# AMReX-Fluids/IAMR

Measured on AMD Instinct MI355X. Metric: cells-advanced/sec, higher is better.
Workload: dtype f64; 1 GPU; TaylorGreen 3D single level, one 256^3 box per GPU in a 1x1x1 arrangement (256x256x256 cells), periodic, nu=1e-4 cfl=0.7 Godunov_PLM be_cn_theta=0.5, full NavierStokes::advance per step

## Files before the change

iamr_amd/csrc/cabi.hip:

```cpp
#include "../../include/iamrx.h"
#include "operators.h"
#include "launch.h"
#include "amrns.h"
#include <string>
#include <cstring>
#include <vector>
#include <map>

using namespace iamrx;

struct iamrx_layout_s { LayoutP p; };
struct iamrx_mf_s { MultiFab mf; };

static thread_local std::string g_err;

#define IAMRX_TRY try {
#define IAMRX_CATCH                                                   \
    return 0; }                                                       \
    catch (const std::exception& e) { g_err = e.what(); return 1; }   \
    catch (...) { g_err = "unknown error"; return 2; }

static Geometry to_geom(const iamrx_geom* g)
{
    Geometry r;
// ... 565 lines not shown
        for (int d = 0; d < 3; ++d) { r[i].lo[d] = b ? b[6 * i + d] : 0; r[i].hi[d] = b ? b[6 * i + 3 + d] : 0; }
    return r;
}

int iamrx_mf_fill_physbc(iamrx_mf m, const iamrx_geom* g, int scomp, int ncomp, const int* bcrec, const double* edlo, const double* edhi)
{
    IAMRX_TRY
    auto bc = to_bcrec(bcrec, ncomp);
    fill_physbc_cc(to_geom(g), m->mf, scomp, ncomp, bc.data(), edlo, edhi);
    IAMRX_CATCH
}

int iamrx_godunov_extrap_vel_to_faces(const iamrx_geom* g, iamrx_mf vel, iamrx_mf force, iamrx_mf ux, iamrx_mf uy, iamrx_mf uz,
                                      double dt, const int* bcrec, int fit, int scheme)
{
    IAMRX_TRY
    auto bc = to_bcrec(bcrec, 3);
    MultiFab* um[3] = {&ux->mf, &uy->mf, &uz->mf};
    godunov_extrap_vel_to_faces(to_geom(g), vel->mf, force ? &force->mf : nullptr, um, dt, bc.data(), fit != 0, scheme);
    IAMRX_CATCH
}

int iamrx_godunov_compute_aofs(const iamrx_geom* g, iamrx_mf aofs, int acomp, iamrx_mf S, int ncomp, iamrx_mf force, iamrx_mf divu,
                               iamrx_mf ux, iamrx_mf uy, iamrx_mf uz, const int* iconserv, double dt, const int* bcrec,
                               int is_velocity, int fit, iamrx_mf ex, iamrx_mf ey, iamrx_mf ez, iamrx_mf fx, iamrx_mf fy, iamrx_mf fz, int scheme)
{
    IAMRX_TRY
    auto bc = to_bcrec(bcrec, ncomp);
    MultiFab* um[3] = {&ux->mf, &uy->mf, &uz->mf};
    MultiFab* ed[3] = {ex ? &ex->mf : nullptr, ey ? &ey->mf : nullptr, ez ? &ez->mf : nullptr};
    MultiFab* fl[3] = {fx ? &fx->mf : nullptr, fy ? &fy->mf : nullptr, fz ? &fz->mf : nullptr};
    godunov_compute_aofs(to_geom(g), aofs->mf, acomp, S->mf, ncomp, force ? &force->mf : nullptr, divu ? &divu->mf : nullptr, um,
                         iconserv, dt, bc.data(), is_velocity != 0, fit != 0, ex ? ed : nullptr, fx ? fl : nullptr, scheme);
    IAMRX_CATCH
}

int iamrx_nodal_residual(const iamrx_geom* g, iamrx_mf out, iamrx_mf phi, iamrx_mf sig, iamrx_mf rhs)
{
    IAMRX_TRY nodal_residual(to_geom(g), out->mf, phi->mf, sig->mf, rhs ? &rhs->mf : nullptr); IAMRX_CATCH
}
int iamrx_nodal_gs_color(const iamrx_geom* g, iamrx_mf phi, iamrx_mf rhs, iamrx_mf sig, int color)
{
    IAMRX_TRY nodal_gs_color(to_geom(g), phi->mf, rhs->mf, sig->mf, color); IAMRX_CATCH
}
int iamrx_nodal_gs_sweep(const iamrx_geom* g, iamrx_mf phi, iamrx_mf rhs, iamrx_mf sig, int fused)
{
    IAMRX_TRY
    Geometry gg = to_geom(g);
    if (fused == 3 || fused == 4) {
        static MultiFab& xb = *new MultiFab();
        if (!xb.defined() || xb.layout != phi->mf.layout || xb.ngrow != phi->mf.ngrow) xb.define(phi->mf.layout, node_type(), 1, phi->mf.ngrow);
        const bool wrap = fused == 4;
        if (wrap && !periodic_wrap_ok(gg, *phi->mf.layout, 4)) throw Error("iamrx_nodal_gs_sweep(4): not a single box spanning a periodic domain");
        const double cs = tune("BENCH_CSIG", 0.0);
        nodal_gs_fused_pass(gg, phi->mf, phi->mf, xb, rhs->mf, sig->mf, 0, wrap, nullptr, cs != 0.0 ? &cs : nullptr);
        nodal_gs_fused_pass(gg, phi->mf, xb, xb, rhs->mf, sig->mf, 1, wrap, nullptr, cs != 0.0 ? &cs : nullptr);
    } else if (fused == 2) {
        if (!nodal_smooth_small(gg, phi->mf, rhs->mf, sig->mf, 1)) throw Error("level does not qualify for the single-workgroup smoother");
        phi->mf.FillBoundary(gg);
    } else if (fused) {
        MultiFab xb(phi->mf.layout, node_type(), 1, phi->mf.ngrow);
        phi->mf.FillBoundary(gg);
        nodal_gs_fused_pass(gg, phi->mf, phi->mf, xb, rhs->mf, sig->mf, 0);
        xb.FillBoundary(gg);
        nodal_gs_fused_pass(gg, phi->mf, xb, xb, rhs->mf, sig->mf, 1);
        MultiFab::Copy(phi->mf, xb, 0, 0, 1, 0);
    } else {
        for (int c = 0; c < 8; ++c) { phi->mf.FillBoundary(gg); nodal_gs_color(gg, phi->mf, rhs->mf, sig->mf, c); }
    }
    IAMRX_CATCH
}
int iamrx_nodal_restrict(iamrx_mf c, iamrx_mf f) { IAMRX_TRY nodal_restrict(c->mf, f->mf); IAMRX_CATCH }
int iamrx_nodal_interp_add(iamrx_mf f, iamrx_mf c, iamrx_mf s) { IAMRX_TRY nodal_interp_add(f->mf, c->mf, s->mf); IAMRX_CATCH }
int iamrx_nodal_divu(const iamrx_geom* g, iamrx_mf rhs, iamrx_mf vel, int vcomp)
{
    IAMRX_TRY
    Geometry gg = to_geom(g);
    DomainBC bc;
    for (int d = 0; d < 3; ++d) bc.lo[d] = bc.hi[d] = gg.periodic[d] ? lo_periodic : lo_neumann;
    bc.maxorder = 2;
    nodal_divu(gg, rhs->mf, vel->mf, vcomp, &bc);
    IAMRX_CATCH
}
int iamrx_nodal_compgrad(const iamrx_geom* g, iamrx_mf gp, iamrx_mf phi)
{
    IAMRX_TRY nodal_mknewu(to_geom(g), nullptr, 0, phi->mf, nullptr, &gp->mf, false); IAMRX_CATCH
}

int iamrx_nodal_projection(const iamrx_geom* g, iamrx_mf vel, int vcomp, iamrx_mf phi, iamrx_mf sig, int sig_comp, const int lobc[3],
                           const int hibc[3], double rel_tol, double abs_tol, const iamrx_mg_opts* o, iamrx_mf gp, int increment_gp,
                           iamrx_mg_stats* st)
{
    IAMRX_TRY
    MGOpts op = to_opts(o);
    MGStats s = nodal_projection(to_geom(g), vel->mf, vcomp, phi->mf, sig->mf, sig_comp, to_bc(lobc, hibc, op.maxorder), rel_tol, abs_tol,
                                 op, gp ? &gp->mf : nullptr, increment_gp != 0);
    from_stats(s, st);
    IAMRX_CATCH
}

int iamrx_nodal_solve(const iamrx_geom* g, iamrx_mf phi, iamrx_mf rhs, iamrx_mf sig, int sig_comp, const int lobc[3], const int hibc[3],
                      double rel_tol, double abs_tol, const iamrx_mg_opts* o, iamrx_mg_stats* st)
{
    IAMRX_TRY
    MGOpts op = to_opts(o);
    NodalMG mg(to_geom(g), phi->mf.layout, to_bc(lobc, hibc, op.maxorder), op);
    mg.setSigma(sig->mf, sig_comp);
    MGStats s = mg.solve(phi->mf, rhs->mf, rel_tol, abs_tol);
    from_stats(s, st);
    IAMRX_CATCH
}

int iamrx_tensor_apply(const iamrx_geom* g, iamrx_mf out, iamrx_mf vel, double a, double b, iamrx_mf acoef, iamrx_mf ex, iamrx_mf ey,
                       iamrx_mf ez, const int* lobc, const int* hibc, int nbc, int maxorder)
{
    IAMRX_TRY
    IAMRX_ASSERT(nbc == 1 || nbc == 3);
    const MultiFab* eta[3] = {&ex->mf, &ey->mf, &ez->mf};
    DomainBC bcs[3];
    for (int n = 0; n < nbc; ++n) bcs[n] = to_bc(lobc + 3 * n, hibc + 3 * n, maxorder);
    tensor_apply(to_geom(g), out->mf, vel->mf, a, b, acoef ? &acoef->mf : nullptr, eta, bcs, nbc);
    IAMRX_CATCH
}

int iamrx_tensor_solve(const iamrx_geom* g, iamrx_mf soln, iamrx_mf rhs, double a, double b, iamrx_mf acoef, iamrx_mf ex, iamrx_mf ey,
                       iamrx_mf ez, const int* lobc, const int* hibc, int nbc, double tol_rel, double tol_abs, const iamrx_mg_opts* o,
                       iamrx_mg_stats* st)
{
    IAMRX_TRY
    IAMRX_ASSERT(nbc == 1 || nbc == 3);
    MGOpts op = to_opts(o);
    const MultiFab* eta[3] = {&ex->mf, &ey->mf, &ez->mf};
    DomainBC bcs[3];
    for (int n = 0; n < nbc; ++n) bcs[n] = to_bc(lobc + 3 * n, hibc + 3 * n, op.maxorder);
    MGStats s = tensor_solve(to_geom(g), soln->mf, rhs->mf, a, b, acoef ? &acoef->mf : nullptr, eta, bcs, nbc, tol_rel, tol_abs, op);
    from_stats(s, st);
    IAMRX_CATCH
}

int iamrx_tensor_extensive_flux(const iamrx_geom* g, iamrx_mf vel, iamrx_mf ex, iamrx_mf ey, iamrx_mf ez, iamrx_mf fx, iamrx_mf fy, iamrx_mf fz,
                                double fac, int add)
{
    IAMRX_TRY
    const MultiFab* eta[3] = {&ex->mf, &ey->mf, &ez->mf};
    MultiFab* fl[3] = {&fx->mf, &fy->mf, &fz->mf};
    tensor_extensive_flux(to_geom(g), vel->mf, eta, fl, fac, add != 0);
    IAMRX_CATCH
}

int iamrx_tensor_apply_cf(const iamrx_geom* g, iamrx_mf out, iamrx_mf vel, double a, double b, iamrx_mf acoef, iamrx_mf ex, iamrx_mf ey,
                          iamrx_mf ez, const int* lobc, const int* hibc, int nbc, int maxorder, iamrx_mf crse_vel, const iamrx_geom* cgeom, int ratio)
{
    IAMRX_TRY
    IAMRX_ASSERT(nbc == 1 || nbc == 3);
    const MultiFab* eta[3] = {&ex->mf, &ey->mf, &ez->mf};
    DomainBC bcs[3];
    for (int n = 0; n < nbc; ++n) bcs[n] = to_bc(lobc + 3 * n, hibc + 3 * n, maxorder);
    Geometry cg = to_geom(cgeom);
    TensorCF cf{crse_vel ? &crse_vel->mf : nullptr, &cg, ratio};
    tensor_apply(to_geom(g), out->mf, vel->mf, a, b, acoef ? &acoef->mf : nullptr, eta, bcs, nbc, &cf);
    IAMRX_CATCH
}

int iamrx_tensor_solve_cf(const iamrx_geom* g, iamrx_mf soln, iamrx_mf rhs, double a, double b, iamrx_mf acoef, iamrx_mf ex, iamrx_mf ey,
                          iamrx_mf ez, const int* lobc, const int* hibc, int nbc, iamrx_mf crse_vel, const iamrx_geom* cgeom, int ratio,
                          double tol_rel, double tol_abs, const iamrx_mg_opts* o, iamrx_mg_stats* st)
// ... 797 lines not shown
```

iamr_amd/csrc/k_basic.hip:

```cpp
#include "kernels.h"
#include "launch.h"

namespace iamrx {

__global__ void __launch_bounds__(256) k_fill(double* __restrict__ p, size_t n, double v)
{
    size_t i = (size_t)blockIdx.x * 256 + threadIdx.x;
    const size_t stride = (size_t)gridDim.x * 256;
    for (; i < n; i += stride) p[i] = v;
}

void launch_fill(double* p, size_t n, double v, hipStream_t s)
{
    if (n == 0) return;
    size_t nb = (n + 255) / 256;
    if (nb > 4096) nb = 4096;
    hipLaunchKernelGGL(k_fill, dim3((unsigned)nb), dim3(256), 0, s, p, n, v);
}

__global__ void __launch_bounds__(256) k_copy_plan(const CopyDesc* __restrict__ descs, const FabD* __restrict__ src,
                                                   const FabD* __restrict__ dst, int scomp, int dcomp, int nc, int add)
{
    const CopyDesc cd = descs[blockIdx.y];
    const int nx = cd.region.len(0), ny = cd.region.len(1);
    const long npts = cd.npts();
    const FabD s = src[cd.src_fab], d = dst[cd.dst_fab];
    for (long q = (long)blockIdx.x * 256 + threadIdx.x; q < npts; q += (long)gridDim.x * 256) {
        const int i = cd.region.lo[0] + (int)(q % nx);
        const long r = q / nx;
        const int j = cd.region.lo[1] + (int)(r % ny);
        const int k = cd.region.lo[2] + cd.kstep * (int)(r / ny);
        if (add) for (int n = 0; n < nc; ++n) d(i, j, k, dcomp + n) += s(i + cd.shift[0], j + cd.shift[1], k + cd.shift[2], scomp + n);
        else for (int n = 0; n < nc; ++n) d(i, j, k, dcomp + n) = s(i + cd.shift[0], j + cd.shift[1], k + cd.shift[2], scomp + n);
    }
}

void launch_copy_plan(const CopyDesc* d, int nd, long maxpts, const FabD* src, const FabD* dst, int scomp, int dcomp, int nc, hipStream_t s, bool add)
{
    if (nd == 0) return;
    long nb = (maxpts + 255) / 256;
    const long cap = nd >= 8 ? 256 : 4096;
    if (nb > cap) nb = cap;
    if (nb < 1) nb = 1;
    hipLaunchKernelGGL(k_copy_plan, dim3((unsigned)nb, (unsigned)nd), dim3(256), 0, s, d, src, dst, scomp, dcomp, nc, add ? 1 : 0);
}

__global__ void __launch_bounds__(256) k_pack(const CopyDesc* __restrict__ descs, const FabD* __restrict__ src,
                                              double* __restrict__ buf, long pts_total, int scomp, int nc)
{
    const CopyDesc cd = descs[blockIdx.y];
    const int nx = cd.region.len(0), ny = cd.region.len(1);
    const long npts = cd.npts();
    const FabD s = src[cd.src_fab];
    for (long q = (long)blockIdx.x * 256 + threadIdx.x; q < npts; q += (long)gridDim.x * 256) {
        const int i = cd.region.lo[0] + (int)(q % nx);
        const long r = q / nx;
        const int j = cd.region.lo[1] + (int)(r % ny);
        const int k = cd.region.lo[2] + cd.kstep * (int)(r / ny);
        for (int n = 0; n < nc; ++n) buf[cd.buf_off + q + pts_total * n] = s(i + cd.shift[0], j + cd.shift[1], k + cd.shift[2], scomp + n);
    }
}

__global__ void __launch_bounds__(256) k_unpack(const CopyDesc* __restrict__ descs, const FabD* __restrict__ dst,
                                                const double* __restrict__ buf, long pts_total, int dcomp, int nc, int add)
{
    const CopyDesc cd = descs[blockIdx.y];
    const int nx = cd.region.len(0), ny = cd.region.len(1);
    const long npts = cd.npts();
    const FabD d = dst[cd.dst_fab];
    for (long q = (long)blockIdx.x * 256 + threadIdx.x; q < npts; q += (long)gridDim.x * 256) {
        const int i = cd.region.lo[0] + (int)(q % nx);
        const long r = q / nx;
        const int j = cd.region.lo[1] + (int)(r % ny);
        const int k = cd.region.lo[2] + cd.kstep * (int)(r / ny);
        if (add) for (int n = 0; n < nc; ++n) d(i, j, k, dcomp + n) += buf[cd.buf_off + q + pts_total * n];
        else for (int n = 0; n < nc; ++n) d(i, j, k, dcomp + n) = buf[cd.buf_off + q + pts_total * n];
    }
}

void launch_pack(const CopyDesc* d, int nd, long maxpts, const FabD* src, double* buf, long pts_total, int scomp, int nc, hipStream_t s)
{
    if (nd == 0) return;
    long nb = (maxpts + 255) / 256; if (nb > 256) nb = 256; if (nb < 1) nb = 1;
    hipLaunchKernelGGL(k_pack, dim3((unsigned)nb, (unsigned)nd), dim3(256), 0, s, d, src, buf, pts_total, scomp, nc);
// ... 339 lines not shown
}

template <bool MASK>
__global__ void __launch_bounds__(256) k_sum_integrated(Tiling t, const BoxD* __restrict__ boxes, const FabD* __restrict__ st, const FabD* __restrict__ cov,
                                                        int rho_comp, int trac_comp, double* __restrict__ partials, int np)
{
    const int fab = tile_fab(t);
    const BoxD b = boxes[fab];
    int i, j, k0, k1;
    double s0 = 0.0, s1 = 0.0, s2 = 0.0;
    if (tile_ijk(t, b, i, j, k0, k1)) {
        const FabD s = st[fab];
        for (int k = k0; k <= k1; ++k) {
            if (MASK && cov[fab](i, j, k) != 0.0) continue;
            const double u = s(i, j, k, 0), v = s(i, j, k, 1), w = s(i, j, k, 2), r = s(i, j, k, rho_comp), q = s(i, j, k, trac_comp);
            s0 += r; s1 += q; s2 += 0.5 * r * (u * u + v * v + w * w);
        }
    }
    const size_t slot = (size_t)blockIdx.y * gridDim.x + blockIdx.x;
    s0 = block_reduce<0>(s0);
    if (threadIdx.x == 0) partials[slot] = s0;
    s1 = block_reduce<0>(s1);
    if (threadIdx.x == 0) partials[(size_t)np + slot] = s1;
    s2 = block_reduce<0>(s2);
    if (threadIdx.x == 0) partials[2 * (size_t)np + slot] = s2;
}

void reduce_sum_integrated(const MultiFab& S, int rho_comp, int trac_comp, const MultiFab* cov, double out[3])
{
    IAMRX_ASSERT(S.type.cell() && (!cov || (cov->type.cell() && cov->layout->id == S.layout->id)));
    out[0] = out[1] = out[2] = 0.0;
    if (S.nlocal() == 0) return;
    auto& ctx = Context::get();
    Tiling t = level_tiling(*S.layout, S.type, 0, 8, true);
    dim3 g = t.grid();
    const int np = (int)(g.x * g.y);
    ctx.ensure_scratch((size_t)3 * np + 16);
    if (cov) hipLaunchKernelGGL((k_sum_integrated<true>), g, Tiling::block(), 0, ctx.stream, t, S.layout->d_boxes, S.d_tab, cov->d_tab, rho_comp, trac_comp, ctx.d_scratch, np);
    else hipLaunchKernelGGL((k_sum_integrated<false>), g, Tiling::block(), 0, ctx.stream, t, S.layout->d_boxes, S.d_tab, (const FabD*)nullptr, rho_comp, trac_comp, ctx.d_scratch, np);
    finish_to_host(0, 3, np, false);
    for (int q = 0; q < 3; ++q) out[q] = ctx.h_scratch[q];
}

void mf_lincomb(MultiFab& dst, double a, const MultiFab& x, double b, const MultiFab& y, int comp, int nc, int ng)
{
    trace_blas_site("lincomb", dst.layout ? dst.layout->local_cells() * nc : 0);
    if (!dst.base) return;
    const FabD *dt = dst.d_tab, *xt = x.d_tab, *yt = y.d_tab;
    for_each_2ph(*dst.layout, dst.type, ng, nc, Context::get().stream,
        [=] __device__(int i, int j, int k, int f, int n) { return a * xt[f](i, j, k, comp + n) + b * yt[f](i, j, k, comp + n); },
        [=] __device__(int i, int j, int k, int f, int n, double v) { dt[f](i, j, k, comp + n) = v; });
}

void mf_saxpy(MultiFab& y, double a, const MultiFab& x, int xcomp, int ycomp, int nc, int ng)
{
    trace_blas_site("saxpy", y.layout ? y.layout->local_cells() * nc : 0);
    if (!y.base) return;
    const FabD *yt = y.d_tab, *xt = x.d_tab;
    for_each_2ph(*y.layout, y.type, ng, nc, Context::get().stream,
        [=] __device__(int i, int j, int k, int f, int n) { return yt[f](i, j, k, ycomp + n) + a * xt[f](i, j, k, xcomp + n); },
        [=] __device__(int i, int j, int k, int f, int n, double v) { yt[f](i, j, k, ycomp + n) = v; });
}

void mf_add_scalar(MultiFab& y, double a, int comp, int nc, int ng)
{
    if (!y.base) return;
    const FabD* yt = y.d_tab;
    for_each(*y.layout, y.type, ng, Context::get().stream, [=] __device__(int i, int j, int k, int f) {
        const FabD yy = yt[f];
        for (int n = 0; n < nc; ++n) yy(i, j, k, comp + n) += a;
    });
}

void mf_mult(MultiFab& y, double a, int comp, int nc, int ng)
{
    trace_blas_site("mult", y.layout ? y.layout->local_cells() * nc : 0);
    if (!y.base) return;
    const FabD* yt = y.d_tab;
    for_each_2ph(*y.layout, y.type, ng, nc, Context::get().stream,
        [=] __device__(int i, int j, int k, int f, int n) { return yt[f](i, j, k, comp + n) * a; },
        [=] __device__(int i, int j, int k, int f, int n, double v) { yt[f](i, j, k, comp + n) = v; });
}

void slab_duplicate(MultiFab& dst, const MultiFab& src)
{
    IAMRX_ASSERT(dst.ncomp == src.ncomp && dst.layout->boxes.size() == src.layout->boxes.size());
    if (dst.nlocal() == 0) return;
    const FabD *dt = dst.d_tab, *st = src.d_tab;
    const int nc = dst.ncomp;
    for_each(*dst.layout, dst.type, 0, Context::get().stream, [=] __device__(int i, int j, int k, int f) {
        const FabD s = st[f];
        for (int n = 0; n < nc; ++n) dt[f](i, j, k, n) = s(i, 0, k, n);
    });
}

}
```

iamr_amd/csrc/k_nodal.hip:

```cpp
#include "kernels.h"
#include <cstring>
#include <type_traits>
#include "launch.h"

namespace iamrx {

struct NodeW { double corner, ex, ey, ez, fx, fy, fz, c; };

static NodeW make_w(const Geometry& g)
{
    const double fx = 1.0 / (g.dx[0] * g.dx[0]) / 36.0, fy = 1.0 / (g.dx[1] * g.dx[1]) / 36.0, fz = 1.0 / (g.dx[2] * g.dx[2]) / 36.0;
    NodeW w;
    w.corner = fx + fy + fz;
    w.ex = -fx + 2.0 * fy + 2.0 * fz;
    w.ey = 2.0 * fx - fy + 2.0 * fz;
    w.ez = 2.0 * fx + 2.0 * fy - fz;
    w.fx = 4.0 * fx - 2.0 * fy - 2.0 * fz;
    w.fy = -2.0 * fx + 4.0 * fy - 2.0 * fz;
    w.fz = -2.0 * fx - 2.0 * fy + 4.0 * fz;
    w.c = -4.0 * (fx + fy + fz);
    return w;
}

__device__ __forceinline__ double node_Ax(const FabD& x, const FabD& s, const NodeW& w, int i, int j, int k, double& s0)
// ... 1300 lines not shown
    long M = 1;
    for (int d = 0; d < 3; ++d) {
        if (b.len(d) < 2 || b.len(d) > 8) return false;
        G.wrap[d] = (g.periodic[d] && b.lo[d] == g.domain.lo[d] && b.hi[d] == g.domain.hi[d]) ? 1 : 0;
        G.m[d] = b.len(d) + (G.wrap[d] ? 0 : 1);
        G.lo[d] = b.lo[d]; G.n[d] = b.len(d);
        G.half_lo[d] = g.half_lo[d]; G.half_hi[d] = g.half_hi[d]; G.dlo[d] = g.domain.lo[d]; G.dhi[d] = g.domain.hi[d];
        M *= G.m[d];
    }
    return M <= NBG_NT;
}

bool nodal_bottom_device_ok_general(const Geometry& g, const Layout& l)
{
    const bool enabled = tune("MG_DEVICE_BOTTOM", 1) != 0 && tune("MG_DEVICE_BOTTOM_GENERAL", 1) != 0;
    NBotGeom G;
    return enabled && nbg_geom(g, l, G);
}

void nodal_bottom_solve_general(const Geometry& g, MultiFab& cor, const MultiFab& res, const MultiFab& sig, const MultiFab* dmask, bool singular,
                                double eps_rel, int maxiter, int nsweeps, int nub, int nuf, int* d_iters)
{
    const Layout& l = *cor.layout;
    NBotGeom G;
    IAMRX_ASSERT(nbg_geom(g, l, G) && sig.ngrow >= 1);
    if (l.nlocal() == 0) return;
    double cnt = 1.0;
    for (int d = 0; d < 3; ++d) cnt *= (double)g.domain.len(d);
    hipLaunchKernelGGL(k_nodal_bottom_g, dim3(1), dim3(NBG_NT), 0, Context::get().stream, cor.d_tab, res.d_tab, sig.d_tab,
                       dmask ? dmask->d_tab : nullptr, make_w(g), G, singular ? 1 : 0, cnt, eps_rel, maxiter, nsweeps, nub, nuf, d_iters);
}

void nodal_jacobi(const Geometry& g, MultiFab& xnew, const MultiFab& x, const MultiFab& rhs, const MultiFab& sig, const MultiFab* dmask)
{
    if (x.nlocal() == 0) return;
    const NodeW w = make_w(g);
    const FabD *nt = xnew.d_tab, *xt = x.d_tab, *rt = rhs.d_tab, *st = sig.d_tab, *dt = dmask ? dmask->d_tab : nullptr;
    for_each(*x.layout, node_type(), 0, Context::get().stream, [=] __device__(int i, int j, int k, int f) {
        if (dt && dt[f](i, j, k) != 0.0) { nt[f](i, j, k) = xt[f](i, j, k); return; }
        double s0;
        const double Ax = node_Ax(xt[f], st[f], w, i, j, k, s0);
        nt[f](i, j, k) = xt[f](i, j, k) + (2. / 3.) * (rt[f](i, j, k) - Ax) / s0;
    });
}

void nodal_zero_masked(MultiFab& mf, const MultiFab& dmask)
{
    if (mf.nlocal() == 0) return;
    const FabD *mt = mf.d_tab, *dt = dmask.d_tab;
    for_each(*mf.layout, node_type(), 0, Context::get().stream, [=] __device__(int i, int j, int k, int f) {
        if (dt[f](i, j, k) != 0.0) mt[f](i, j, k) = 0.0;
    });
}

void nodal_build_dmask(const Geometry& g, MultiFab& dm, const MultiFab& cov, const DomainBC& bc)
{
    if (dm.nlocal() == 0) return;
    const FabD *dt = dm.d_tab, *ct = cov.d_tab;
    int lo[3], hi[3], tlo[3], thi[3];
    for (int d = 0; d < 3; ++d) {
        lo[d] = g.domain.lo[d]; hi[d] = g.domain.hi[d];
        tlo[d] = g.periodic[d] ? 0 : bc.lo[d]; thi[d] = g.periodic[d] ? 0 : bc.hi[d];
    }
    const int l0 = lo[0], l1 = lo[1], l2 = lo[2], h0 = hi[0], h1 = hi[1], h2 = hi[2];
    const int a0 = tlo[0], a1 = tlo[1], a2 = tlo[2], b0 = thi[0], b1 = thi[1], b2 = thi[2];
    for_each(*dm.layout, node_type(), 0, Context::get().stream, [=] __device__(int i, int j, int k, int f) {
        const FabD c = ct[f];
        bool in = true;
        for (int q = 0; q < 8; ++q) {
            int ci = i - 1 + (q & 1), cj = j - 1 + ((q >> 1) & 1), ck = k - 1 + ((q >> 2) & 1);
            bool out = false;
            if (ci < l0) { if (a0 == lo_neumann) ci = 2 * l0 - 1 - ci; else if (a0 != 0) out = true; }
            else if (ci > h0) { if (b0 == lo_neumann) ci = 2 * h0 + 1 - ci; else if (b0 != 0) out = true; }
            if (cj < l1) { if (a1 == lo_neumann) cj = 2 * l1 - 1 - cj; else if (a1 != 0) out = true; }
            else if (cj > h1) { if (b1 == lo_neumann) cj = 2 * h1 + 1 - cj; else if (b1 != 0) out = true; }
            if (ck < l2) { if (a2 == lo_neumann) ck = 2 * l2 - 1 - ck; else if (a2 != 0) out = true; }
            else if (ck > h2) { if (b2 == lo_neumann) ck = 2 * h2 + 1 - ck; else if (b2 != 0) out = true; }
            if (out || c(ci, cj, ck) == 0.0) in = false;
        }
        dt[f](i, j, k) = in ? 0.0 : 1.0;
    });
}

void nodal_restrict(MultiFab& crse, const MultiFab& fine)
{
    if (crse.nlocal() == 0) return;
    const FabD *ct = crse.d_tab, *ft = fine.d_tab;
    for_each(*crse.layout, node_type(), 0, Context::get().stream, [=] __device__(int i, int j, int k, int f) {
        const FabD fa = ft[f];
        const int ii = 2 * i, jj = 2 * j, kk = 2 * k;
        double s = 0.0;
        for (int dk = -1; dk <= 1; ++dk)
            for (int dj = -1; dj <= 1; ++dj)
                for (int di = -1; di <= 1; ++di) {
                    const double w = (di == 0 ? 2. : 1.) * (dj == 0 ? 2. : 1.) * (dk == 0 ? 2. : 1.);
                    s += w * fa(ii + di, jj + dj, kk + dk);
                }
        ct[f](i, j, k) = s * (1. / 64.);
    });
}

#ifndef IAMRX_INTERP_EXP
#define IAMRX_INTERP_EXP 0
#endif
__device__ __forceinline__ double w_side(const FabD& s, int i, int j, int k, int d, int side)
{
    int lo[3] = {i - 1, j - 1, k - 1}, hi[3] = {i, j, k};
    lo[d] = hi[d] = (d == 0 ? i : (d == 1 ? j : k)) - 1 + side;
    double r = 0.0;
    for (int c = lo[2]; c <= hi[2]; ++c) for (int b = lo[1]; b <= hi[1]; ++b) for (int a = lo[0]; a <= hi[0]; ++a) r += s(a, b, c);
    return r;
}
__device__ __forceinline__ double interp_line(const FabD& c, const FabD& s, int i, int j, int k, int ic, int jc, int kc, int d)
{
    const double w1 = w_side(s, i, j, k, d, 0), w2 = w_side(s, i, j, k, d, 1);
    const double c2 = c(ic + (d == 0), jc + (d == 1), kc + (d == 2));
    return (c(ic, jc, kc) * w1 + c2 * w2) / (w1 + w2);
}
__device__ __forceinline__ double interp_face(const FabD& c, const FabD& s, int i, int j, int k, int ic, int jc, int kc, int d1, int d2)
{
    const double w1 = w_side(s, i, j, k, d1, 0), w2 = w_side(s, i, j, k, d1, 1), w3 = w_side(s, i, j, k, d2, 0), w4 = w_side(s, i, j, k, d2, 1);
    const int e1[3] = {d1 == 0, d1 == 1, d1 == 2}, e2[3] = {d2 == 0, d2 == 1, d2 == 2};
    double r = 0.0;
    r += w1 * interp_line(c, s, i - e1[0], j - e1[1], k - e1[2], ic, jc, kc, d2);
    r += w2 * interp_line(c, s, i + e1[0], j + e1[1], k + e1[2], ic + e1[0], jc + e1[1], kc + e1[2], d2);
    r += w3 * interp_line(c, s, i - e2[0], j - e2[1], k - e2[2], ic, jc, kc, d1);
    r += w4 * interp_line(c, s, i + e2[0], j + e2[1], k + e2[2], ic + e2[0], jc + e2[1], kc + e2[2], d1);
    return r / (w1 + w2 + w3 + w4);
}

template <class SA>
__device__ __forceinline__ void side_weights(const SA& s, int i, int j, int k, double w[6])
{
#if IAMRX_INTERP_EXP & 1
    for (int t = 0; t < 6; ++t) w[t] = 1.0 + 1e-3 * t;
    return;
#endif
    double g[2][2][2];
#pragma unroll
    for (int c = 0; c < 2; ++c)
#pragma unroll
        for (int b = 0; b < 2; ++b)
#pragma unroll
            for (int a = 0; a < 2; ++a) g[c][b][a] = s(i - 1 + a, j - 1 + b, k - 1 + c);
#pragma unroll
    for (int t = 0; t < 2; ++t) {
        w[t] = ((g[0][0][t] + g[0][1][t]) + g[1][0][t]) + g[1][1][t];
        w[2 + t] = ((g[0][t][0] + g[0][t][1]) + g[1][t][0]) + g[1][t][1];
        w[4 + t] = ((g[t][0][0] + g[t][0][1]) + g[t][1][0]) + g[t][1][1];
    }
}

template <int PX, int PY, int PZ, int CX, int CY, int CZ, class SA>
__device__ __forceinline__ void interp_class(double (*T)[2 * CY + 1][2 * CX + 1], const FabD& c, const SA& s, int fi0, int fj0, int fk0,
                                             int nhi0, int nhi1, int nhi2, int tid)
{
    constexpr int NX = PX ? CX : CX + 1, NY = PY ? CY : CY + 1, NZ = PZ ? CZ : CZ + 1, CLS = PX + PY + PZ;
    for (int idx = tid; idx < NX * NY * NZ; idx += 256) {
        const int lx = 2 * (idx % NX) + PX, q = idx / NX, ly = 2 * (q % NY) + PY, lz = 2 * (q / NY) + PZ;
        const int i = fi0 + lx, j = fj0 + ly, k = fk0 + lz;
        if (i > nhi0 || j > nhi1 || k > nhi2) continue;
        if (CLS == 0) { T[lz][ly][lx] = c(i >> 1, j >> 1, k >> 1); continue; }
        double w[6];
        side_weights(s, i, j, k, w);
        if (CLS == 1) {
            constexpr int d = PX ? 0 : (PY ? 1 : 2);
            const double w1 = w[2 * d], w2 = w[2 * d + 1];
            T[lz][ly][lx] = (IAMRX_INTERP_EXP & 4) ? (T[lz - PZ][ly - PY][lx - PX] * w1 + T[lz + PZ][ly + PY][lx + PX] * w2) * (w1 + w2) : (T[lz - PZ][ly - PY][lx - PX] * w1 + T[lz + PZ][ly + PY][lx + PX] * w2) / (w1 + w2);
        } else if (CLS == 2) {
            constexpr int d1 = PX ? 0 : 1, d2 = PZ ? 2 : 1;
// ... 16 lines not shown
__global__ void __launch_bounds__(256) k_nodal_interp_lds(const BoxD* __restrict__ fboxes, const FabD* __restrict__ ft, const FabD* __restrict__ ct,
    const FabD* __restrict__ st, int ntx, int nty)
{
    constexpr int FX = 2 * CX + 1, FY = 2 * CY + 1, FZ = 2 * CZ + 1, NF = FX * FY * FZ;
    __shared__ double T[FZ][FY][FX];
    const int fab = blockIdx.y;
    const BoxD vb = fboxes[fab];
    const int bid = blockIdx.x;
    const int tix = bid % ntx, r1 = bid / ntx, tiy = r1 % nty, tiz = r1 / nty;
    const int nhi0 = vb.hi[0] + 1, nhi1 = vb.hi[1] + 1, nhi2 = vb.hi[2] + 1;
    const int fi0 = vb.lo[0] + tix * 2 * CX, fj0 = vb.lo[1] + tiy * 2 * CY, fk0 = vb.lo[2] + tiz * 2 * CZ;
    if (fi0 >= nhi0 || fj0 >= nhi1 || fk0 >= nhi2) return;
    const FabD c = ct[fab], sg = st[fab], fa = ft[fab];
    const int tid = threadIdx.x;
    const FabD& s = sg;
#define IAMRX_ICLS(PX, PY, PZ) interp_class<PX, PY, PZ, CX, CY, CZ>(T, c, s, fi0, fj0, fk0, nhi0, nhi1, nhi2, tid)
    IAMRX_ICLS(0, 0, 0);
    __syncthreads();
    IAMRX_ICLS(1, 0, 0); IAMRX_ICLS(0, 1, 0); IAMRX_ICLS(0, 0, 1);
    __syncthreads();
    IAMRX_ICLS(1, 1, 0); IAMRX_ICLS(1, 0, 1); IAMRX_ICLS(0, 1, 1);
    __syncthreads();
    IAMRX_ICLS(1, 1, 1);
    __syncthreads();
#undef IAMRX_ICLS
    for (int idx = tid; idx < NF; idx += 256) {
        const int lx = idx % FX, q = idx / FX, ly = q % FY, lz = q / FY;
        const int i = fi0 + lx, j = fj0 + ly, k = fk0 + lz;
        if (i > nhi0 || j > nhi1 || k > nhi2) continue;
        if ((lx == 2 * CX && i != nhi0) || (ly == 2 * CY && j != nhi1) || (lz == 2 * CZ && k != nhi2)) continue;
        if (IAMRX_INTERP_EXP & 2) fa(i, j, k) = T[lz][ly][lx]; else fa(i, j, k) += T[lz][ly][lx];
    }
}

static bool nodal_interp_lds_enabled()
{
    const bool on = tune("NODAL_INTERP_LDS", 1) != 0;
    return on;
}

void nodal_interp_add(MultiFab& fine, const MultiFab& crse, const MultiFab& sig_fine)
{
    if (fine.nlocal() == 0) return;
    if (nodal_interp_lds_enabled()) {
        const Layout& l = *fine.layout;
        bool even = true;
        for (int d = 0; d < 3; ++d) even = even && l.all_lo_even[d];
        if (even) {
            constexpr int CX = 16, CY = 4, CZ = 4;
            const int ntx = (l.max_len[0] + 2 * CX - 1) / (2 * CX), nty = (l.max_len[1] + 2 * CY - 1) / (2 * CY), ntz = (l.max_len[2] + 2 * CZ - 1) / (2 * CZ);
            dim3 grid((unsigned)(ntx * nty * ntz), (unsigned)l.nlocal());
            hipLaunchKernelGGL((k_nodal_interp_lds<CX, CY, CZ>), grid, dim3(256), 0, Context::get().stream, l.d_boxes, fine.d_tab, crse.d_tab, sig_fine.d_tab, ntx, nty);
            return;
        }
    }
    const FabD *ft = fine.d_tab, *ct = crse.d_tab, *st = sig_fine.d_tab;
    const BoxD* fb = fine.layout->d_boxes;
    for_each(*crse.layout, node_type(), 0, Context::get().stream, [=] __device__(int ic, int jc, int kc, int f) {
        const FabD c = ct[f], s = st[f], fa = ft[f];
        const BoxD vb = fb[f];
        const int nhi0 = vb.hi[0] + 1, nhi1 = vb.hi[1] + 1, nhi2 = vb.hi[2] + 1;
        const int i0 = 2 * ic, j0 = 2 * jc, k0 = 2 * kc;
        const bool xi = i0 + 1 <= nhi0, xj = j0 + 1 <= nhi1, xk = k0 + 1 <= nhi2;
        fa(i0, j0, k0) += c(ic, jc, kc);
        if (xi) fa(i0 + 1, j0, k0) += interp_line(c, s, i0 + 1, j0, k0, ic, jc, kc, 0);
        if (xj) fa(i0, j0 + 1, k0) += interp_line(c, s, i0, j0 + 1, k0, ic, jc, kc, 1);
        if (xk) fa(i0, j0, k0 + 1) += interp_line(c, s, i0, j0, k0 + 1, ic, jc, kc, 2);
        if (xi && xj) fa(i0 + 1, j0 + 1, k0) += interp_face(c, s, i0 + 1, j0 + 1, k0, ic, jc, kc, 0, 1);
        if (xi && xk) fa(i0 + 1, j0, k0 + 1) += interp_face(c, s, i0 + 1, j0, k0 + 1, ic, jc, kc, 0, 2);
        if (xj && xk) fa(i0, j0 + 1, k0 + 1) += interp_face(c, s, i0, j0 + 1, k0 + 1, ic, jc, kc, 1, 2);
        if (xi && xj && xk) {
            const int i = i0 + 1, j = j0 + 1, k = k0 + 1;
            double w[6];
            for (int d = 0; d < 3; ++d) { w[2 * d] = w_side(s, i, j, k, d, 0); w[2 * d + 1] = w_side(s, i, j, k, d, 1); }
            const double v = (w[0] * interp_face(c, s, i - 1, j, k, ic, jc, kc, 1, 2) + w[1] * interp_face(c, s, i + 1, j, k, ic + 1, jc, kc, 1, 2)
               + w[2] * interp_face(c, s, i, j - 1, k, ic, jc, kc, 0, 2) + w[3] * interp_face(c, s, i, j + 1, k, ic, jc + 1, kc, 0, 2)
               + w[4] * interp_face(c, s, i, j, k - 1, ic, jc, kc, 0, 1) + w[5] * interp_face(c, s, i, j, k + 1, ic, jc, kc + 1, 0, 1))
              / (w[0] + w[1] + w[2] + w[3] + w[4] + w[5]);
            fa(i, j, k) += v;
        }
    });
}

void nodal_divu(const Geometry& g, MultiFab& rhs, const MultiFab& vel, int vcomp, const DomainBC* bc)
{
    if (rhs.nlocal() == 0) return;
    const FabD *rt = rhs.d_tab, *vt = vel.d_tab;
    const double fx = 0.25 / g.dx[0], fy = 0.25 / g.dx[1], fz = 0.25 / g.dx[2];
    int wl[3], wh[3], il[3], ih[3];
    for (int d = 0; d < 3; ++d) {
        wl[d] = (bc && !g.periodic[d] && bc->lo[d] == lo_neumann) ? 1 : 0;
        wh[d] = (bc && !g.periodic[d] && bc->hi[d] == lo_neumann) ? 1 : 0;
        il[d] = (bc && !g.periodic[d] && bc->lo[d] == lo_inflow) ? 1 : 0;
        ih[d] = (bc && !g.periodic[d] && bc->hi[d] == lo_inflow) ? 1 : 0;
    }
    const int wl0 = wl[0], wl1 = wl[1], wl2 = wl[2], wh0 = wh[0], wh1 = wh[1], wh2 = wh[2];
    const int il0 = il[0], il1 = il[1], il2 = il[2], ih0 = ih[0], ih1 = ih[1], ih2 = ih[2];
    const int dl0 = g.domain.lo[0], dl1 = g.domain.lo[1], dl2 = g.domain.lo[2], dh0 = g.domain.hi[0], dh1 = g.domain.hi[1], dh2 = g.domain.hi[2];
    for_each(*rhs.layout, node_type(), 0, Context::get().stream, [=] __device__(int i, int j, int k, int f) {
        const FabD v = vt[f];
        double sx = 0.0, sy = 0.0, sz = 0.0;
        for (int cz = 0; cz < 2; ++cz) for (int cy = 0; cy < 2; ++cy) for (int cx = 0; cx < 2; ++cx) {
            const int ci = i - 1 + cx, cj = j - 1 + cy, ck = k - 1 + cz;
            const bool outside = (wl0 && ci < dl0) || (wh0 && ci > dh0) || (wl1 && cj < dl1) || (wh1 && cj > dh1) || (wl2 && ck < dl2) || (wh2 && ck > dh2);
            const bool in0 = (il0 && ci < dl0) || (ih0 && ci > dh0), in1 = (il1 && cj < dl1) || (ih1 && cj > dh1), in2 = (il2 && ck < dl2) || (ih2 && ck > dh2);
            sx += (cx ? 1.0 : -1.0) * ((outside || in1 || in2) ? 0.0 : v(ci, cj, ck, vcomp));
            sy += (cy ? 1.0 : -1.0) * ((outside || in0 || in2) ? 0.0 : v(ci, cj, ck, vcomp + 1));
            sz += (cz ? 1.0 : -1.0) * ((outside || in0 || in1) ? 0.0 : v(ci, cj, ck, vcomp + 2));
        }
        double r = 0.0;
        r += fx * sx; r += fy * sy; r += fz * sz;
        if ((wl0 || il0) && i == dl0) r *= 2.0;
        if ((wh0 || ih0) && i == dh0 + 1) r *= 2.0;
        if ((wl1 || il1) && j == dl1) r *= 2.0;
        if ((wh1 || ih1) && j == dh1 + 1) r *= 2.0;
        if ((wl2 || il2) && k == dl2) r *= 2.0;
        if ((wh2 || ih2) && k == dh2 + 1) r *= 2.0;
        rt[f](i, j, k) = r;
    });
}

void nodal_mknewu(const Geometry& g, MultiFab* vel, int vcomp, const MultiFab& phi, const MultiFab* sig, MultiFab* gp, bool gp_increment)
{
    if (phi.nlocal() == 0) return;
    const FabD* pt = phi.d_tab;
    const FabD* vt = vel ? vel->d_tab : nullptr;
    const FabD* st = sig ? sig->d_tab : nullptr;
    const FabD* gt = gp ? gp->d_tab : nullptr;
    const double fac[3] = {0.25 / g.dx[0], 0.25 / g.dx[1], 0.25 / g.dx[2]};
    const double f0 = fac[0], f1 = fac[1], f2 = fac[2];
    for_each(*phi.layout, cell_type(), 0, Context::get().stream, [=] __device__(int i, int j, int k, int f) {
        const FabD p = pt[f];
        double s[3] = {0.0, 0.0, 0.0};
        for (int nz = 0; nz < 2; ++nz) for (int ny = 0; ny < 2; ++ny) for (int nx = 0; nx < 2; ++nx) {
            const double v = p(i + nx, j + ny, k + nz);
            s[0] += (nx ? 1.0 : -1.0) * v;
            s[1] += (ny ? 1.0 : -1.0) * v;
            s[2] += (nz ? 1.0 : -1.0) * v;
        }
        const double gr[3] = {f0 * s[0], f1 * s[1], f2 * s[2]};
        if (vt) {
            const double sg = st[f](i, j, k);
            const double fc[3] = {f0, f1, f2};
            for (int d = 0; d < 3; ++d) vt[f](i, j, k, vcomp + d) -= sg * fc[d] * s[d];
        }
        if (gt) for (int d = 0; d < 3; ++d) { if (gp_increment) gt[f](i, j, k, d) += gr[d]; else gt[f](i, j, k, d) = gr[d]; }
    });
}

}
```

iamr_amd/csrc/kernels.h:

```cpp
#pragma once
#include "core.h"
#include "mf.h"

namespace iamrx {

void launch_fill(double* p, size_t n, double v, hipStream_t s);
void launch_copy_plan(const CopyDesc* d, int nd, long maxpts, const FabD* src, const FabD* dst, int scomp, int dcomp, int nc, hipStream_t s, bool add = false);
void launch_pack(const CopyDesc* d, int nd, long maxpts, const FabD* src, double* buf, long pts_total, int scomp, int nc, hipStream_t s);
void launch_unpack(const CopyDesc* d, int nd, long maxpts, const FabD* dst, const double* buf, long pts_total, int dcomp, int nc, hipStream_t s, bool add = false);
void launch_copy_plan_w(const CopyDesc* d, const int2* w, int nw, const FabD* src, const FabD* dst, int scomp, int dcomp, int nc, hipStream_t s, bool add);
void launch_pack_w(const CopyDesc* d, const int2* w, int nw, const FabD* src, double* buf, long pts_total, int scomp, int nc, hipStream_t s);
void launch_unpack_w(const CopyDesc* d, const int2* w, int nw, const FabD* dst, const double* buf, long pts_total, int dcomp, int nc, hipStream_t s, bool add);
double reduce_norm0(const MultiFab& mf, int comp, int nc, int ng, bool global = false);
void reduce_norm0_comps(const MultiFab& mf, int comp, int nc, int ng, double* out, bool global = false);
void reduce_minmax(const MultiFab& mf, int comp, int ng, double& mn, double& mx, bool global = true);
double reduce_sum_unique(const MultiFab& mf, int comp, const Geometry& g, bool global = false);
void reduce_sum_integrated(const MultiFab& S, int rho_comp, int trac_comp, const MultiFab* cov, double out[3]);
void reduce_dots(int nout, const MultiFab* const* x, const MultiFab* const* y, int comp, int nc, const Geometry& g, double* out, bool local = false);
void reduce_dots_dev(int nout, const MultiFab* const* x, const MultiFab* const* y, int comp, int nc, const Geometry& g, double* d_out, bool local = false);
enum { PROBE_NODAL_GS4 = 0, PROBE_ABEC_GSRB = 1, PROBE_GOD_Z = 2, PROBE_PRED_Z = 3, PROBE_COUNT = 4 };
void kernel_probe_start(int which, long min_points, int stride);
void kernel_probe_stop(int which, double* total_ms, long* launches);
void kernel_probes_pause(bool on);
bool kernel_probe_begin(int which, long points);
void kernel_probe_end(int which);
void gs4_probe_start(long min_nodes, int stride);
void gs4_probe_stop(double* total_ms, long* launches);
void mf_lincomb(MultiFab& dst, double a, const MultiFab& x, double b, const MultiFab& y, int comp, int nc, int ng);
void mf_saxpy(MultiFab& y, double a, const MultiFab& x, int xcomp, int ycomp, int nc, int ng);
void mf_add_scalar(MultiFab& y, double a, int comp, int nc, int ng);
void mf_mult(MultiFab& y, double a, int comp, int nc, int ng);

void stats_accumulate(MultiFab& avg, const MultiFab& S, int vcomp, double dt_avg, double t_sum, bool fluct);
void stats_derive_vel_avg(MultiFab& out, int ocomp, const MultiFab& avg, double t_mean, double t_fluct);

struct DomainBC;
void fill_physbc_cc(const Geometry& g, MultiFab& mf, int scomp, int ncomp, const BCRec* bc, const double* extdir_lo, const double* extdir_hi);

void nodal_reflect_bc(const Geometry& g, MultiFab& mf, const DomainBC& bc, hipStream_t on = nullptr);
void cc_mirror_bc(const Geometry& g, MultiFab& mf);

struct AbecCoef {
    double alpha, beta;
    const MultiFab* a;
    const MultiFab* b[3];
    int tensor;
    int tensor_eta = 0;
    const MultiFab* sig = nullptr;
    int sig_comp = 0;
    double sig_scale = 1.0;
    int b_uniform = 0;
    double bu[3] = {0.0, 0.0, 0.0};
};
bool mf_uniform_value(const MultiFab& m, double* v);
bool tensor_residual_fused(const Geometry& g, const AbecCoef& c, MultiFab& out, const MultiFab& vel, const MultiFab* rhs, double* norm_out);
struct DomainBC {
    int lo[3], hi[3];
    int maxorder;
};
struct CfTab { double c[3][3][4]; int maxorder; };
CfTab cf_make_tab(const double loc[3], const double dx[3], int maxorder);
void cf_build_mask(const Geometry& g, MultiFab& cfm);
void cf_fill_ghosts(MultiFab& phi, const MultiFab& cfm, const CfTab& tab, bool inhomog, const MultiFab* bcval, bool edges = false);
void cf_interp_edges(MultiFab& bcval, const MultiFab& cpatch, const MultiFab& cfm, int ratio, const Geometry& cgeom);
void cf_interp_bndry(MultiFab& bcval, const MultiFab& cpatch, const MultiFab& cfm, int ratio);
struct AbecLevel {
    const std::vector<BoxD>* boxes = nullptr;
    int nlocal = 0, max_len[3] = {0, 0, 0};
    int ncomp = 1;
    int phi_ngrow = 1, rhs_ngrow = 0, sig_ngrow = 0, a_ngrow = 0;
    bool sig = false, b_uniform = false, has_a = false, tensor_eta = false;
    bool tensor = false;
    int b_ncomp = 1;
    int nbc = 0;
    const DomainBC* bcs = nullptr;
    bool has_cf = false;
    bool finest = true;
};
AbecLevel abec_level(const AbecCoef& c, const MultiFab& phi, int rhs_ngrow, int nbc, const DomainBC* bcs, bool has_cf = false, bool finest = true);
struct AbecColourForm {
    enum Kernel { GENERAL, GSRB1, GSRB2, GSRB2_PER_COMP } kernel = GENERAL;
    int mode = 0;
    int np = 1;
    bool gen_mc = false;
    int gen_mode = 0;
    bool has_cf = false, maintain = false, allcf = false;
    bool wrap = false;
    bool walls_inkernel = false;
    bool zero_ok = false;
};
struct AbecSmoothPlan {
    enum Path { COLOUR, RB_BOX, RB_CF, RB_NBR, FUSED_SHELL } path = COLOUR;
    AbecColourForm colour;
    int nw = 16;
    bool nbr_splits = false;
    bool zero_first = false;
    int ncomp = 1, phi_ngrow = 1, rhs_ngrow = 0;
    bool sweep_kernel() const { return path == RB_BOX || path == RB_CF || path == RB_NBR; }
    bool made_for(const MultiFab& phi, const MultiFab& rhs) const { return phi.ncomp == ncomp && phi.ngrow == phi_ngrow && rhs.ngrow == rhs_ngrow; }
};
AbecSmoothPlan abec_smooth_plan(const Geometry& g, const AbecLevel& lv);
AbecColourForm abec_colour_form(const Geometry& g, const AbecLevel& lv, bool wrap = false, bool walls_inkernel = false);
void abec_gsrb(const Geometry& g, const AbecCoef& c, const AbecColourForm& f, MultiFab& phi, const MultiFab& rhs, int redblack, double omega,
               const DomainBC* bcs, int nbc, bool shell_only = false, bool phi_is_zero = false, const MultiFab* cfm = nullptr, const CfTab* cftab = nullptr);
bool abec_tail_ok(const Geometry& gF, const Layout& lF, const Geometry& gC, const Layout& lC, const AbecCoef& cF, const DomainBC* bcs, int nbc, int ncomp);
void abec_tail_solve(const Geometry& gF, const AbecCoef& cF, MultiFab& corF, const MultiFab& resF, const Geometry& gC, const AbecCoef& cC,
                     const DomainBC& bc, bool singular, double eps_rel, int maxiter, int nub, int nuf, int nu1, int nu2, double omega, int* d_iters);
bool abec_residual_reads_no_ghosts(const Geometry& g, const AbecCoef& c, const MultiFab& out, const MultiFab& phi, const MultiFab& rhs, bool restrict_form);
bool abec_resid_restrict_ok(const AbecCoef& c, const MultiFab& phi, const MultiFab& rhs);
void abec_resid_restrict(const Geometry& g, const AbecCoef& c, MultiFab& crse, const MultiFab& phi, const MultiFab& rhs);
void abec_gsrb_rb(const Geometry& g, const AbecCoef& c, const AbecSmoothPlan& p, const MultiFab& pin, MultiFab& pout, const MultiFab& rhs, double omega,
                  bool zero, const DomainBC* bcs = nullptr, int nbc = 0, const CfTab* cf = nullptr, bool acc = false);
void abec_gsrb_rb_nbr(const Geometry& g, const AbecCoef& c, const AbecSmoothPlan& p, MultiFab& pin, MultiFab& pout, const MultiFab& rhs, double omega,
                      bool zero, const DomainBC* bcs, int nbc, int sel = 0, hipStream_t on = nullptr, bool acc = false);
bool abec_gsrb_rb_ok(const Geometry& g, const AbecCoef& c, const MultiFab& phi, int nbc, const DomainBC* bcs = nullptr);
bool abec_gsrb_rb_cf_ok(const Geometry& g, const AbecCoef& c, const MultiFab& phi);
bool abec_gsrb_rb_nbr_ok(const Geometry& g, const AbecCoef& c, const MultiFab& phi, const MultiFab& rhs, int nbc, const DomainBC* bcs);
bool abec_gsrb_rb_nbr_level_ok(const Geometry& g, const Layout& l, int ncomp, bool sig_form, bool has_a, int nbc, const DomainBC* bcs);
void abec_gsrb_fused(const Geometry& g, const AbecCoef& c, const MultiFab& phi_in, MultiFab& phi_out, const MultiFab& rhs, double omega,
                     const DomainBC* bcs, int nbc);
void abec_residual(const Geometry& g, const AbecCoef& c, MultiFab& out, const MultiFab& phi, const MultiFab* rhs, double* norm_out = nullptr);
bool abec_bottom_device_ok(const Geometry& g, const Layout& l, const DomainBC* bcs, int nbc, int ncomp, bool cf = false);
void abec_bottom_solve(const Geometry& g, const AbecCoef& c, MultiFab& cor, const MultiFab& res, const DomainBC& bc, bool singular,
                       double eps_rel, int maxiter, int nub, int nuf, double omega, int* d_iters, const CfTab* cftab = nullptr);
void abec_apply_domain_bc(const Geometry& g, MultiFab& phi, const DomainBC& bc, bool inhomog, const MultiFab* bcval, int comp0 = 0, int ncomp = -1);
void abec_apply_domain_bc_percomp(const Geometry& g, MultiFab& phi, const DomainBC* bcs, int ncomp, bool inhomog, const MultiFab* bcval);
void cc_restrict(MultiFab& crse, const MultiFab& fine);
void cc_prolong_add(MultiFab& fine, const MultiFab& crse);
void face_avgdown(MultiFab& crse, const MultiFab& fine, int dir);
void abec_flux(const Geometry& g, const AbecCoef& c, const MultiFab& phi, MultiFab* const flux[3], MultiFab* const add_to[3]);
void mac_rhs(const Geometry& g, MultiFab& rhs, const MultiFab* const umac[3], const MultiFab* S);
void mac_bcoef(MultiFab* const b[3], const MultiFab& rho, int rho_comp, double scale);
void mac_divergence(const Geometry& g, MultiFab& div, const MultiFab* const umac[3]);

void godunov_extrap_vel_to_faces(const Geometry& g, const MultiFab& vel, const MultiFab* force, MultiFab* const umac[3],
                                 double dt, const BCRec* bc, bool use_forces_in_trans, int scheme = 0);
void godunov_compute_aofs(const Geometry& g, MultiFab& aofs, int acomp, const MultiFab& S, int ncomp, const MultiFab* force,
                          const MultiFab* divu, MultiFab* const umac[3], const int* iconserv, double dt, const BCRec* bc,
                          bool is_velocity, bool use_forces_in_trans, MultiFab* const edge_out[3], MultiFab* const flux_out[3], int scheme = 0);


bool nodal_residual(const Geometry& g, MultiFab& out, const MultiFab& x, const MultiFab& sig, const MultiFab* rhs, double* norm_out = nullptr);
void nodal_gs_color(const Geometry& g, MultiFab& x, const MultiFab& rhs, const MultiFab& sig, int color, const MultiFab* dmask = nullptr);
void nodal_gs_fused_pass(const Geometry& g, const MultiFab& xc, const MultiFab& xn, MultiFab& xo, const MultiFab& rhs, const MultiFab& sig, int kpar,
                         bool wrap = false, const MultiFab* dmask = nullptr, const double* csig = nullptr, int zero_flags = 0, int refl = 0,
                         int sel = 0, hipStream_t on = nullptr);
bool nodal_gsr_splits(const MultiFab& x, const MultiFab& rhs, const MultiFab* dmask);
bool nodal_gsr_applies(const MultiFab& x, const MultiFab& rhs, const MultiFab* dmask);
void nodal_zero_masked(MultiFab& mf, const MultiFab& dmask);
void nodal_build_dmask(const Geometry& g, MultiFab& dm, const MultiFab& cov, const DomainBC& bc);
bool periodic_wrap_ok(const Geometry& g, const Layout& l, int min_len);
bool nodal_wrap_or_reflect_ok(const Geometry& g, const Layout& l, const DomainBC& bc, int min_len, int* refl);
bool nodal_smooth_small(const Geometry& g, MultiFab& x, const MultiFab& rhs, const MultiFab& sig, int nsweeps);
void nodal_jacobi(const Geometry& g, MultiFab& xnew, const MultiFab& x, const MultiFab& rhs, const MultiFab& sig, const MultiFab* dmask = nullptr);
void nodal_restrict(MultiFab& crse, const MultiFab& fine);
void nodal_interp_add(MultiFab& fine, const MultiFab& crse, const MultiFab& sig_fine);
void nodal_divu(const Geometry& g, MultiFab& rhs, const MultiFab& vel, int vcomp, const DomainBC* bc);
void nodal_mknewu(const Geometry& g, MultiFab* vel, int vcomp, const MultiFab& phi, const MultiFab* sig, MultiFab* gp, bool gp_increment);

void tensor_bcoef(MultiFab& b3, const MultiFab& eta, int dir);
void tensor_extensive_flux(const Geometry& g, const MultiFab& vel, const MultiFab* const eta[3], MultiFab* const flux[3], double fac, bool add);
void tensor_cross_terms_sub(const Geometry& g, const AbecCoef& c, MultiFab& out, const MultiFab& vel, double sign, unsigned long long* normout = nullptr);
void fill_tensor_corners(const Geometry& g, MultiFab& phi, const DomainBC& bc, bool inhomog, const MultiFab* bcval, int comp0 = 0, int ncomp = -1);

void les_mut(const Geometry& g, const MultiFab& vel, int vcomp, int model, double Cs, double base, MultiFab* const mu[3]);

}
```

iamr_amd/csrc/mlmg.h:

```cpp
#pragma once
#include <functional>
#include "mf.h"
#include "kernels.h"
#include <vector>
#include <memory>

namespace iamrx {

inline bool mg_stalled_at_floor(const std::vector<double>& hist, double r0, double target, bool fast)
{
    const size_t n = hist.size();
    if (n == 0 || !(hist[n - 1] <= 10.0 * target)) return false;
    if (n >= 4 && hist[n - 1] > 0.9 * hist[n - 4]) return true;
    if (!fast || n < 2) return false;
    const double last = hist[n - 1] / hist[n - 2];
    double best = 1.0, prev = r0;
    for (size_t i = 0; i + 1 < n; ++i) { if (prev > 0.0) best = std::min(best, hist[i] / prev); prev = hist[i]; }
    return last > 0.5 && best < 0.2;
}


struct MGOpts {
    int nu1 = 2, nu2 = 2, nuf = 8, nub = 0;
    int max_iters = 200;
// ... 79 lines not shown
public:
    CellMG(const Geometry& g, LayoutP layout, int ncomp, const DomainBC& bc, const MGOpts& o);
    void setScalars(double alpha, double beta) { m_alpha = alpha; m_beta = beta; }
    void setACoeffs(const MultiFab* a) { m_a0 = a; }
    void setBCoeffs(const MultiFab* const b[3]) { for (int d = 0; d < 3; ++d) m_b0[d] = b[d]; }
    void setBCoeffsFromCell(const MultiFab* sig, int comp, double scale) { m_sig = sig; m_sig_comp = comp; m_sig_scale = scale; }
    void setTensor(bool t) { m_tensor = t; }
    void setTensorEta(bool t) { m_tensor_eta = t; }
    void setDomainBCs(const DomainBC* bcs, int n) { m_bcn.assign(bcs, bcs + n); }
    void setCoarseFineBC(const MultiFab* crse, const Geometry& cgeom, int ratio) { m_cf = true; m_crse = crse; m_cgeom = cgeom; m_ratio = ratio; }
    void prepare();
    void prepareBoundary();
    void fillBoundaryData(MultiFab& phi);
    MGStats solve(MultiFab& phi, const MultiFab& rhs, double rtol, double atol);
    void apply(MultiFab& out, MultiFab& phi);
    void fluxes(MultiFab& phi, MultiFab* const flux[3], MultiFab* const add_to[3]);
    int nlevels() const { return (int)m_lev.size(); }
    AbecCoef coef(int l) const;
    AbecCoef smoother_coef(int l) const;
    const Geometry& geom(int l) const { return m_lev[l].g; }
    void applyBC(int l, MultiFab& phi, bool inhomog, const MultiFab* bcval, bool corners = true);
    void smooth(int l, bool skip_fill, bool cf_ghosts_current = false, bool sol_is_zero = false);
    void smooth_n(int l, int nsweeps, bool skip_first_fill, bool sol_is_zero = false, MultiFab* acc = nullptr);
    void vcycle(MGStats& st);
    MultiFab& res(int l) { return m_lev[l].res; }
    MultiFab& cor(int l) { return m_lev[l].cor; }

private:
    struct Level : MGLevel {
        MultiFab a, b[3];
        MultiFab cor, res, rescor;
        MultiFab buf;
        AbecSmoothPlan plan;
        MultiFab cfm;
        CfTab cftab;
    };
    int bicgstab(int l, MultiFab& sol, const MultiFab& rhs, double eps_rel, double eps_abs, int& niters);
    void bottom_solve(MGStats& st);
    template <class Sweep> void pingpong(MultiFab& sol, MultiFab& buf, int nsweeps, bool sol_is_zero, MultiFab* acc, Sweep sweep);
    bool tail_fused() const;
    void cf_bcval(MultiFab& bcval);
    void prepare_cf(int l);
    void subtract_mean(int l, MultiFab& mf);
    Geometry m_g;
    int m_ncomp;
    std::vector<DomainBC> m_bcn;
    MGOpts m_o;
    double m_alpha = 0.0, m_beta = 1.0;
    const MultiFab* m_a0 = nullptr;
    const MultiFab* m_b0[3] = {nullptr, nullptr, nullptr};
    bool m_buni = false;
    bool m_buni_coarse = false;
    double m_bu[3] = {0.0, 0.0, 0.0};
    const MultiFab* m_sig = nullptr;
    int m_sig_comp = 0;
    double m_sig_scale = 1.0;
    bool m_tensor = false;
    bool m_tensor_eta = false;
    bool m_singular = false;
    bool m_bottom_dev = false;
    MultiFab* m_acc = nullptr;
    bool m_acc_done = false;
    bool m_bottom_direct = false;
    const double* m_dB = nullptr;
    std::shared_ptr<double> m_dBh;
    int m_dN = 0;
    void bottom_direct_prepare();
    void bottom_direct_solve();
    double m_dd_rho = 0.0;
    int m_dd_sweeps = 0;
    bool m_nbr = false;
    MultiFab m_sig2, m_a1;
    bool m_cf = false;
    const MultiFab* m_crse = nullptr;
    Geometry m_cgeom;
    int m_ratio = 2;
    std::vector<Level> m_lev;
};

class NodalMG {
public:
    NodalMG(const Geometry& g, LayoutP layout, const DomainBC& bc, const MGOpts& o);
    void setSigma(const MultiFab& sig, int comp);
    MGStats solve(MultiFab& phi, const MultiFab& rhs, double rtol, double atol);
    int nlevels() const { return (int)m_lev.size(); }
    bool masked() const { return m_masked; }
    const MultiFab* dmask(int l) const { return m_lev[l].dmask(); }
    const MultiFab& sigma(int l) const { return m_lev[l].sig; }
    const Geometry& geom(int l) const { return m_lev[l].g; }
    void smooth(int l, MultiFab& x, const MultiFab& rhs, bool x_is_zero = false, bool leave_ghosts = false);
    void residual(int l, MultiFab& r, MultiFab& x, const MultiFab& b, double* norm = nullptr, bool x_filled = false);
    void vcycle(MGStats& st);
    void vcycle_correction(MultiFab& e, const MultiFab& r, MGStats& st);
    void vcycle_correction_inplace(MGStats& st);
    MultiFab& res(int l) { return m_lev[l].res; }
    MultiFab& cor(int l) { return m_lev[l].cor; }

private:
    struct Level : MGLevel {
        MultiFab sig;
        MultiFab cor, res, rescor;
        MultiFab tmp;
        MultiFab xb;
        MultiFab dm;
        const MultiFab* dmask() const { return dm.defined() ? &dm : nullptr; }
    };
    int bicgstab(int l, MultiFab& sol, const MultiFab& rhs, double eps_rel, double eps_abs, int& niters);
    bool bottom_on_device();
    void subtract_mean(int l, MultiFab& mf);
    void fillbc(int l, MultiFab& x, int kpar = -1, hipStream_t on = nullptr);
    Geometry m_g;
    DomainBC m_bc;
    MGOpts m_o;
    bool m_singular = true;
    bool m_csig = false;
    double m_csig_val = 0.0;
    bool m_masked = false;
    std::vector<Level> m_lev;
};

}
```

iamr_amd/csrc/navierstokes.hip:

```cpp
#include "operators.h"
#include "launch.h"
#include <cmath>
#include <chrono>

namespace iamrx {

namespace {
struct SectionTimer {
    NavierStokes& ns; int idx; bool on;
    std::chrono::steady_clock::time_point t0;
    SectionTimer(NavierStokes& n, int i) : ns(n), idx(i), on(n.profile_sections)
    {
        if (on) { Context::get().sync(); t0 = std::chrono::steady_clock::now(); }
    }
    ~SectionTimer()
    {
        if (on) { Context::get().sync(); ns.t_sections[idx] += std::chrono::duration<double, std::milli>(std::chrono::steady_clock::now() - t0).count(); }
    }
};
}

static LayoutP level_work_layout(const Geometry& geom, const LayoutP& lay)
{
    return (lay && lay->total_cells() == geom.domain.npts()) ? coalesce_layout(lay) : lay;
// ... 1025 lines not shown
        fillpatch(tmp, from, Xvel, 3, bc_vel);
        MultiFab::Copy(U, tmp, 0, Xvel, 3, 1);
    };
    if (theta != 1.0 && !reuse) refill(So, So);
    MultiFab co, cn;
    DiffusionCrse dc{nullptr, nullptr, level > 0 ? &crse->g : nullptr, ratio};
    if (level > 0) {
        if (theta != 1.0 && !reuse) { crse_state_at(co, st_old, Xvel, 3); dc.crse_old = &co; }
        crse_state_at(cn, st_new, Xvel, 3); dc.crse_new = &cn;
    }
    st_visc = diffuse_tensor_velocity(g, &So, Sn, Density, dt_, theta, rho_half, p.do_mom_diff ? 3 : 1, reuse ? &m_visc_old : nullptr, en, ep, bc_visc,
                                      level > 0 ? &dc : nullptr, want_flux ? tfp : nullptr, p.visc_tol, o, [&](MultiFab& U) { refill(U, U); });
    if (want_flux)
        for (int d = 0; d < 3; ++d) {
            if (level > 0) reg_visc->FineAdd(tflux[d], d, 0, Xvel, 3, dt_);
            if (fine) fine->reg_visc->CrseInit(tflux[d], d, 0, Xvel, 3, -dt_, false);
        }
}

void NavierStokes::level_project(double dt_)
{
    SectionTimer tm(*this, 5);
    MultiFab& Sn = S[inew];
    MultiFab& Pn = P[pnew];
    const bool warm = tune("WARM_START", 1) != 0;
    const bool extrap = tune("WARM_EXTRAP", 1) != 0;
    if (level == 0) {
        const double dto = pt_old[1] - pt_old[0];
        if (warm && extrap && nstep >= 2 && !initial_iter && !initial_step && dto > 0.0) mf_lincomb(Pn, 1.0 + dt_ / dto, P[1 - pnew], -dt_ / dto, Pn, 0, 1, 0);
        else if (warm) MultiFab::Copy(Pn, P[1 - pnew], 0, 0, 1, 0);
        else Pn.setVal(0.0, 0, 1, 0);
    }
    else {
        const double tp = 0.5 * (pt_new[0] + pt_new[1]);
        const double teps = 1.e-3 * std::abs(crse->pt_new[0] - crse->pt_old[0]);
        const MultiFab* Pc;
        if (tp >= crse->pt_new[0] - teps && tp <= crse->pt_new[1] + teps) Pc = &crse->P[crse->pnew];
        else if (tp >= crse->pt_old[0] - teps && tp <= crse->pt_old[1] + teps) Pc = &crse->P[1 - crse->pnew];
        else throw Error("iamrx NavierStokes::level_project: the coarse level has no pressure at the requested time");
        node_interp_from_crse(Pn, *Pc, crse->g, ratio, nullptr, false);
        const FabD *pt = Pn.d_tab, *po = P[1 - pnew].d_tab;
        const BoxD* vb = layout->d_boxes;
        const bool use_old = warm;
        for_each(*layout, node_type(), 0, Context::get().stream, [=] __device__(int i, int j, int k, int f) {
            const BoxD b = vb[f];
            if (i > b.lo[0] && i <= b.hi[0] && j > b.lo[1] && j <= b.hi[1] && k > b.lo[2] && k <= b.hi[2]) pt[f](i, j, k) = use_old ? (double)po[f](i, j, k) : 0.0;
        });
    }
    MultiFab sig(layout, cell_type(), 1, 1);
    {
        const FabD *nt = Sn.d_tab, *gt = Gp[1 - pnew].d_tab, *ht = rho_half.d_tab, *st = sig.d_tab;
        const BoxD* vb = layout->d_boxes;
        const double rdt = 1.0 / dt_;
        for_each(*layout, cell_type(), 1, Context::get().stream, [=] __device__(int i, int j, int k, int f) {
            const BoxD b = vb[f];
            const bool valid = i >= b.lo[0] && i <= b.hi[0] && j >= b.lo[1] && j <= b.hi[1] && k >= b.lo[2] && k <= b.hi[2];
            double rh = 1.0;
            if (valid) { rh = ht[f](i, j, k, 0); st[f](i, j, k, 0) = 1.0 / rh; }
            for (int n = 0; n < 3; ++n) {
                double v = nt[f](i, j, k, n) * rdt;
                if (valid) v += gt[f](i, j, k, n) / rh;
                nt[f](i, j, k, n) = v;
            }
        });
    }
    set_outflow_bcs(Pn, rho_half, 0);
    set_inflow_ghosts(Sn, 1.0 / dt_);
    const bool want_crse = fine != nullptr, want_fine = level > 0 && iteration == ncycle;
    MultiFab vold;
    if (want_crse || want_fine) {
        Sn.FillBoundary(g, Xvel, 3);
        vold.define(layout, cell_type(), 3, 1);
        MultiFab::Copy(vold, Sn, Xvel, 0, 3, 1);
    }
    MultiFab rhv, rhcc;
    if (have_divu) {
        rhv.define(layout, cell_type(), 1, 0);
        MultiFab::Copy(rhv, Sn, Divu, 0, 1, 0);
        mf_mult(rhv, 1.0 / dt_, 0, 1, 0);
        mf_mult(rhv, -1.0, 0, 1, 0);
        rhcc = make_rhcc(g, rhv, 0, 1.0, nullptr);
    }
    const MultiFab* rv = have_divu ? &rhv : nullptr;
    st_nodal = nodal_projection(g, Sn, Xvel, Pn, sig, 0, bc_nodal, p.proj_tol, p.proj_abs_tol, o, &Gp[pnew], false, have_divu ? &rhcc : nullptr);
    fill_gradp_bc();
    if (want_crse) {
        MultiFab r = amr_sync_resid(*this, vold, Pn, sig, true, rv);
        fine->sync_reg->CrseInit(r, 1.0);
    }
    if (want_fine) {
        MultiFab r = amr_sync_resid(*this, vold, Pn, sig, false, rv);
        sync_reg->FineAdd(r, 1.0 / (double)ncycle);
    }
    mf_mult(Sn, dt_, Xvel, 3, 1);
}

void NavierStokes::set_inflow_ghosts(MultiFab& vel, double scale)
{
    for (int d = 0; d < 3; ++d) {
        if (g.periodic[d]) continue;
        for (int side = 0; side < 2; ++side) {
            if ((side == 0 ? bc_nodal.lo[d] : bc_nodal.hi[d]) != lo_inflow) continue;
            const double uin = (side == 0 ? ed_vel_lo[d * 3 + d] : ed_vel_hi[d * 3 + d]) * scale;
            const int face = side == 0 ? g.domain.lo[d] - 1 : g.domain.hi[d] + 1;
            const FabD* vt = vel.d_tab;
            const int dd = d;
            for_each(*layout, cell_type(), 1, Context::get().stream, [=] __device__(int i, int j, int k, int f) {
                const int idx = dd == 0 ? i : (dd == 1 ? j : k);
                if (idx == face) vt[f](i, j, k, Xvel + dd) = uin;
            });
        }
    }
}

void NavierStokes::initial_velocity_project()
{
    if (p.init_vel_iter <= 0) { P[1 - pnew].setVal(0.0); Gp[1 - pnew].setVal(0.0); return; }
    for (int iter = 0; iter < p.init_vel_iter; ++iter) {
        MultiFab& phi = P[1 - pnew];
        phi.setVal(0.0);
        MultiFab sig(layout, cell_type(), 1, 1);
        sig.setVal(1.0);
        set_inflow_ghosts(S[inew], 1.0);
        MultiFab rhcc;
        if (have_divu) rhcc = make_rhcc(g, S[inew], Divu, -1.0, nullptr);
        st_nodal = nodal_projection(g, S[inew], Xvel, phi, sig, 0, bc_nodal, p.proj_tol, p.proj_abs_tol, o, &Gp[pnew], false, have_divu ? &rhcc : nullptr);
        for (int q = 0; q < 2; ++q) { P[q].setVal(0.0); Gp[q].setVal(0.0); }
    }
}

void NavierStokes::initial_sync_project(double dt_)
{
    MultiFab& phi = P[1 - pnew];
    phi.setVal(0.0);
    MultiFab& Sn = S[inew];
    MultiFab& So = S[1 - inew];
    {
        const double dt_inv = 1. / dt_;
        const FabD *nt = Sn.d_tab, *ot = So.d_tab;
        for_each(*layout, cell_type(), 0, Context::get().stream, [=] __device__(int i, int j, int k, int f) {
            for (int n = 0; n < 3; ++n) nt[f](i, j, k, n) = (nt[f](i, j, k, n) - ot[f](i, j, k, n)) * dt_inv;
        });
    }
    MultiFab sig(layout, cell_type(), 1, 1);
    {
        const FabD *st = sig.d_tab, *ht = rho_half.d_tab;
        for_each(*layout, cell_type(), 0, Context::get().stream, [=] __device__(int i, int j, int k, int f) {
            st[f](i, j, k, 0) = 1.0 / ht[f](i, j, k, 0);
        });
    }
    set_inflow_ghosts(Sn, 0.0);
    MultiFab rhcc;
    if (have_divu) {
        MultiFab d(layout, cell_type(), 1, 0);
        MultiFab::Copy(d, Sn, Divu, 0, 1, 0);
        mf_saxpy(d, -1.0, So, Divu, 0, 1, 0);
        mf_mult(d, 1.0 / dt_, 0, 1, 0);
        rhcc = make_rhcc(g, d, 0, -1.0, nullptr);
    }
    st_nodal = nodal_projection(g, Sn, Xvel, phi, sig, 0, bc_nodal, p.proj_tol, p.proj_abs_tol, o, &Gp[pnew], true, have_divu ? &rhcc : nullptr);
    fill_gradp_bc();
    mf_saxpy(P[pnew], 1.0, phi, 0, 0, 1, 1);
}

double NavierStokes::advance(double dt_, int iteration_, int ncycle_)
{
    advance_setup(dt_, iteration_, ncycle_);
    m_in_advance = true; m_visc_old_valid = false; m_eta_n_valid = false;
    const double dt_test = predict_velocity(dt_);
    mac_project(dt_);
    const bool fused_adv = tune("FUSED_ADVECTION", 1) != 0;
    if (fused_adv) advection_all(dt_);
    else { velocity_advection(dt_); scalar_advection(dt_); }
    scalar_update_rho(dt_);
    scalar_update_tracers(dt_);
    scalar_diffusion_update(dt_);
    if (have_divu) {
// ... 179 lines not shown
```

iamr_amd/csrc/nodalmg.hip:

```cpp
#include "mlmg.h"
#include "launch.h"
#include "krylov.h"
#include <chrono>
#include <cmath>
#include <cstdlib>

namespace iamrx {

void nodal_restrict(MultiFab& crse, const MultiFab& fine);
void nodal_interp_add(MultiFab& fine, const MultiFab& crse, const MultiFab& sig_fine);

static bool nodal_fused() { return tune("NODAL_FUSED", 1) != 0; }
static bool nodal_small() { return tune("NODAL_SMALL", 1) != 0; }
bool nodal_smooth_small(const Geometry& g, MultiFab& x, const MultiFab& rhs, const MultiFab& sig, int nsweeps);
bool nodal_bottom_device_ok(const Geometry& g, const Layout& l);
void nodal_bottom_solve(const Geometry& g, MultiFab& cor, const MultiFab& res, const MultiFab& sig, bool singular, double eps_rel, int maxiter,
                        int nsweeps, int nub, int nuf, int* d_iters);
bool nodal_bottom_device_ok_general(const Geometry& g, const Layout& l);
void nodal_bottom_solve_general(const Geometry& g, MultiFab& cor, const MultiFab& res, const MultiFab& sig, const MultiFab* dmask, bool singular,
                                double eps_rel, int maxiter, int nsweeps, int nub, int nuf, int* d_iters);
static long nodal_unknowns(const Geometry& g)
{
    long n = 1;
    for (int d = 0; d < 3; ++d) n *= g.domain.len(d) + (g.periodic[d] ? 0 : 1);
    return n;
}

NodalMG::NodalMG(const Geometry& g, LayoutP layout, const DomainBC& bc_in, const MGOpts& o) : m_g(g), m_bc(bc_in), m_o(o)
{
    ProfScope ps_prof_("nmg_ctor");
    for (int d = 0; d < 3; ++d) { if (m_bc.lo[d] == lo_inflow) m_bc.lo[d] = lo_neumann; if (m_bc.hi[d] == lo_inflow) m_bc.hi[d] = lo_neumann; }
    const DomainBC& bc = m_bc;
    for (int d = 0; d < 3; ++d) {
        if (!g.periodic[d])
            for (int t : {bc.lo[d], bc.hi[d]})
                if (t != lo_neumann && t != lo_dirichlet) throw Error("iamrx NodalMG: domain boundaries must be periodic, Neumann (wall / inflow) or Dirichlet (outflow)");
        m_g.half_lo[d] = (!g.periodic[d] && bc.lo[d] == lo_neumann) ? 1 : 0;
        m_g.half_hi[d] = (!g.periodic[d] && bc.hi[d] == lo_neumann) ? 1 : 0;
    }
    m_lev.resize(1);
    m_lev[0].g = m_g;
    m_lev[0].layout = std::move(layout);
    while ((int)m_lev.size() <= m_o.max_coarsening_level) {
        Level& f = m_lev.back();
        if (m_o.device_bottom && m_o.nodal_smoother == 0 && !m_o.bottom_smoother_only &&
            (nodal_bottom_device_ok(f.g, *f.layout) || nodal_bottom_device_ok_general(f.g, *f.layout))) break;
        Level c;
        if (!mg_coarsen_level(f, m_o, c)) break;
        m_lev.push_back(std::move(c));
    }
    for (auto& L : m_lev) {
        if (L.agg) L.tmp_d.define(L.dist, node_type(), 1, 1);
        if (L.slab) L.vres.define(L.virt, node_type(), 1, 0);
        const int ng = nodal_fused() ? 4 : 1;
        L.sig.define(L.layout, cell_type(), 1, ng);
        L.sig.setVal(0.0);
        L.cor.define(L.layout, node_type(), 1, ng);
        L.res.define(L.layout, node_type(), 1, ng);
        L.rescor.define(L.layout, node_type(), 1, 1);
        L.cor.setVal(0.0); L.res.setVal(0.0); L.rescor.setVal(0.0);
    }
    bool need_mask = false;
    for (int d = 0; d < 3; ++d) if (!g.periodic[d] && (bc.lo[d] == lo_dirichlet || bc.hi[d] == lo_dirichlet)) need_mask = true;
    if (m_lev[0].layout->total_cells() != g.domain.npts()) need_mask = true;
    for (auto& L : m_lev) {
        if (!need_mask) break;
        MultiFab cov(L.layout, cell_type(), 1, 1);
        cov.setVal(0.0);
        mf_add_scalar(cov, 1.0, 0, 1, 0);
        cov.FillBoundary(L.g);
        const int ng = L.cor.ngrow;
        L.dm.define(L.layout, node_type(), 1, ng);
        L.dm.setVal(1.0);
        nodal_build_dmask(L.g, L.dm, cov, m_bc);
        if (L.dm.norm0(0, 1, 0) == 0.0) L.dm = MultiFab();
        else {
            m_masked = true;
            L.dm.FillBoundary(L.g);
            nodal_reflect_bc(L.g, L.dm, m_bc);
        }
    }
    if (m_masked) {
        m_singular = false;
        for (auto& L : m_lev) IAMRX_ASSERT(L.dm.defined());
    }
}

void NodalMG::setSigma(const MultiFab& sig, int comp)
{
    ProfScope ps_prof_("nmg_setsigma");
    MultiFab::Copy(m_lev[0].sig, sig, comp, 0, 1, 0);
    m_lev[0].sig.FillBoundary(m_lev[0].g);
    cc_mirror_bc(m_lev[0].g, m_lev[0].sig);
    for (size_t l = 1; l < m_lev.size(); ++l) {
        {
            Level& C = m_lev[l];
            MultiFab sd, sv;
            if (C.agg) sd.define(C.dist, cell_type(), 1, 0);
            if (C.slab) sv.define(C.virt, cell_type(), 1, 0);
            mg_restrict_to(C, C.sig, sd, sv, [&](MultiFab& target) { cc_restrict(target, m_lev[l - 1].sig); });
        }
        m_lev[l].sig.FillBoundary(m_lev[l].g);
        cc_mirror_bc(m_lev[l].g, m_lev[l].sig);
    }
    const bool csig_on = tune("NODAL_CSIG", 1) != 0;
    m_csig = false;
    if (csig_on && !m_masked) {
        double smin, smax;
        reduce_minmax(m_lev[0].sig, 0, 0, smin, smax);
        if (smax > 0.0 && smin == smax) { m_csig = true; m_csig_val = smax; }
    }
}

void NodalMG::fillbc(int l, MultiFab& x, int kpar, hipStream_t on)
{
    const int ngv[3] = {x.ngrow, x.ngrow, 1};
    x.FillBoundary(m_lev[l].g, 0, x.ncomp, ngv, kpar, on);
    nodal_reflect_bc(m_lev[l].g, x, m_bc, on);
}

void NodalMG::smooth(int l, MultiFab& x, const MultiFab& rhs, bool x_is_zero, bool leave_ghosts)
{
    Level& L = m_lev[l];
    const int zs_mode = (int)tune("NODAL_ZERO_START", 1);
    int zs_refl = 0;
    const bool zero_start = x_is_zero && m_o.nodal_smoother == 0 && nodal_fused() && zs_mode != 0 && nodal_gsr_applies(x, rhs, L.dmask()) &&
                            (zs_mode != 2 || (!L.dmask() && nodal_wrap_or_reflect_ok(L.g, *L.layout, m_bc, 4, &zs_refl)));
    if (x_is_zero && !zero_start) x.setVal(0.0);
    const MultiFab* dmk = L.dmask();
    if (!dmk && m_o.nodal_smoother == 0 && nodal_small() && nodal_smooth_small(L.g, x, rhs, L.sig, m_o.nodal_sweeps)) {
        fillbc(l, x);
        return;
    }
    if (m_o.nodal_smoother == 0 && nodal_fused()) {
        if (!L.xb.defined() || L.xb.ngrow != x.ngrow) L.xb.define(L.layout, node_type(), 1, x.ngrow);
        int refl = 0;
        const bool wrap = !dmk && nodal_wrap_or_reflect_ok(L.g, *L.layout, m_bc, 4, &refl);
        if (!wrap) {
            if (&rhs == &L.res) { if (!L.res_filled) { fillbc(l, L.res); L.res_filled = true; } }
            else fillbc(l, const_cast<MultiFab&>(rhs));
        }
        MultiFab* a = &x;
        MultiFab* b = &L.xb;
        const bool par_fill = tune("NODAL_PARITY_FILL", 1) != 0;
        auto& ctx = Context::get();
        const int ov_mode = (int)tune("HALO_OVERLAP", 1);
        bool overlap = false;
// ... 77 lines not shown
{
    Level& B = m_lev.back();
    if (!(m_o.device_bottom && m_o.nodal_smoother == 0 && !m_o.bottom_smoother_only)) return false;
    return (!B.dmask() && nodal_bottom_device_ok(B.g, *B.layout)) || nodal_bottom_device_ok_general(B.g, *B.layout);
}

void NodalMG::vcycle(MGStats& st)
{
    const int nl = (int)m_lev.size();
    for (int l = 0; l < nl - 1; ++l) {
        Level& L = m_lev[l];
        if (m_o.nodal_nu1 <= 0) L.cor.setVal(0.0);
        for (int i = 0; i < m_o.nodal_nu1; ++i) smooth(l, L.cor, L.res, i == 0);
        residual(l, L.rescor, L.cor, L.res, nullptr, m_o.nodal_nu1 > 0);
        fillbc(l, L.rescor);
        Level& C = m_lev[l + 1];
        mg_restrict_to(C, C.res, C.tmp_d, C.vres, [&](MultiFab& target) { nodal_restrict(target, L.rescor); });
        m_lev[l + 1].res_filled = false;
        if (m_lev[l + 1].dmask()) nodal_zero_masked(m_lev[l + 1].res, m_lev[l + 1].dm);
    }
    {
        const int l = nl - 1;
        Level& B = m_lev[l];
        B.cor.setVal(0.0);
        if (m_o.bottom_smoother_only) {
            for (int i = 0; i < m_o.nuf; ++i) smooth(l, B.cor, B.res);
        } else if (bottom_on_device()) {
            const int maxiter = krylov_maxiter(m_o.bottom_maxiter, nodal_unknowns(B.g));
            if (!B.dmask() && nodal_bottom_device_ok(B.g, *B.layout))
                nodal_bottom_solve(B.g, B.cor, B.res, B.sig, m_singular, m_o.bottom_reltol, maxiter, m_o.nodal_sweeps, m_o.nub, m_o.nuf,
                                   mg_bottom_iters_dev());
            else
                nodal_bottom_solve_general(B.g, B.cor, B.res, B.sig, B.dmask(), m_singular, m_o.bottom_reltol, maxiter, m_o.nodal_sweeps, m_o.nub,
                                           m_o.nuf, mg_bottom_iters_dev());
        } else {
            MultiFab rb(B.layout, node_type(), 1, 0);
            MultiFab::Copy(rb, B.res, 0, 0, 1, 0);
            if (m_singular) subtract_mean(l, rb);
            int nit = 0;
            const int ret = bicgstab(l, B.cor, rb, m_o.bottom_reltol, -1.0, nit);
            st.bottom_iters_total += nit;
            if (ret != 0) {
                B.cor.setVal(0.0);
                for (int i = 0; i < m_o.nuf; ++i) smooth(l, B.cor, B.res);
            }
            const int nn = ret == 0 ? m_o.nub : m_o.nuf;
            for (int i = 0; i < nn; ++i) smooth(l, B.cor, B.res);
        }
    }
    for (int l = nl - 2; l >= 0; --l) {
        Level& L = m_lev[l];
        if (l + 1 == nl - 1 || m_o.nodal_nu2 <= 0) fillbc(l + 1, m_lev[l + 1].cor);
        nodal_interp_add(L.cor, mg_correction_of(m_lev[l + 1], m_lev[l + 1].cor, 1), L.sig);
        if (L.dmask()) nodal_zero_masked(L.cor, L.dm);
        for (int i = 0; i < m_o.nodal_nu2; ++i) smooth(l, L.cor, L.res, false, l == 0 && i == m_o.nodal_nu2 - 1);
    }
}

void NodalMG::vcycle_correction(MultiFab& e, const MultiFab& r, MGStats& st)
{
    Level& L0 = m_lev[0];
    MultiFab::Copy(L0.res, r, 0, 0, 1, 0);
    if (L0.dmask()) nodal_zero_masked(L0.res, L0.dm);
    if (m_singular) subtract_mean(0, L0.res);
    L0.res_filled = false;
    vcycle(st);
    MultiFab::Copy(e, L0.cor, 0, 0, 1, 0);
    e.FillBoundary(L0.g);
    nodal_reflect_bc(L0.g, e, m_bc);
}

void NodalMG::vcycle_correction_inplace(MGStats& st)
{
    Level& L0 = m_lev[0];
    if (L0.dmask()) nodal_zero_masked(L0.res, L0.dm);
    if (m_singular) subtract_mean(0, L0.res);
    L0.res_filled = false;
    vcycle(st);
    const int ngv[3] = {1, 1, 1};
    L0.cor.FillBoundary(L0.g, 0, 1, ngv, -1);
    nodal_reflect_bc(L0.g, L0.cor, m_bc);
}

MGStats NodalMG::solve(MultiFab& phi, const MultiFab& rhs_in, double rtol, double atol)
{
    ProfScope ps_prof_("nmg_solve");
    auto& ctx = Context::get();
    MGStats st;
    st.nlevels = (int)m_lev.size();
    Level& L0 = m_lev[0];
    MultiFab rhs(L0.layout, node_type(), 1, 0);
    MultiFab::Copy(rhs, rhs_in, 0, 0, 1, 0);
    if (L0.dmask()) nodal_zero_masked(rhs, L0.dm);
    if (m_singular) subtract_mean(0, rhs);
    residual(0, L0.res, phi, rhs, &st.resnorm0);
    L0.res_filled = false;
    st.rhsnorm0 = rhs.norm0(0, 1, 0);
    const double max_norm = st.rhsnorm0 >= st.resnorm0 ? st.rhsnorm0 : st.resnorm0;
    if (!std::isfinite(max_norm)) throw Error("iamrx nodal MLMG: the right-hand side or the initial residual is not finite");
    const double res_target = std::max(atol, std::max(rtol, 1.e-16) * max_norm);
    st.resnorm = st.resnorm0;
    if (m_o.verbose) printf("iamrx nodal MLMG: rhs %.6e resid0 %.6e levels %d (fused sweep %d, single-workgroup coarse smoother %d, ghost width %d)\n",
                            st.rhsnorm0, st.resnorm0, st.nlevels, (int)nodal_fused(), (int)nodal_small(), L0.cor.ngrow);
    double vc_ms = 0.0;
    cycle_timer().used = 0;
    const bool bdev = bottom_on_device();
    if (bdev) IAMRX_HIP_CHECK(hipMemsetAsync(mg_bottom_iters_dev(), 0, sizeof(int), ctx.stream));
    if (m_o.fixed_iters <= 0 && st.resnorm0 <= res_target) st.converged = 1;
    else {
        const int maxit = m_o.fixed_iters > 0 ? m_o.fixed_iters : m_o.max_iters;
        std::vector<double> hist;
        for (int iter = 0; iter < maxit; ++iter) {
            const bool all_per = L0.g.periodic[0] && L0.g.periodic[1] && L0.g.periodic[2] && !L0.dmask();
            if (m_singular && (!all_per || tune("MG_RES_MEAN", 0) != 0)) { subtract_mean(0, L0.res); L0.res_filled = false; }
            cycle_timer().mark(ctx.stream);
            vcycle(st);
            cycle_timer().mark(ctx.stream);
            mf_saxpy(phi, 1.0, L0.cor, 0, 0, 1, 0);
            residual(0, L0.res, phi, rhs, &st.resnorm);
            L0.res_filled = false;
            st.iters = iter + 1;
            if (m_o.verbose) printf("iamrx nodal MLMG: iter %d resid %.6e\n", iter + 1, st.resnorm);
            if (m_o.fixed_iters <= 0 && st.resnorm <= res_target) { st.converged = 1; break; }
            if (!(st.resnorm < 1.e20 * max_norm)) throw Error("iamrx nodal MLMG: failing to converge (residual blow-up)");
            hist.push_back(st.resnorm);
            if (m_o.fixed_iters <= 0 && mg_stalled_at_floor(hist, st.resnorm0, res_target, tune("MG_STALL_FAST", 1) != 0)) {
                st.converged = 2;
                fprintf(stderr, "iamrx nodal MLMG: WARNING: residual %.3e stalled at the round-off floor above the target %.3e after %d cycles; accepted (converged = 2)\n",
                        st.resnorm, res_target, st.iters);
                break;
            }
        }
        if (m_o.fixed_iters <= 0 && !st.converged) throw Error("iamrx nodal MLMG: failed to converge after max_iters");
    }
    vc_ms = cycle_timer().total_ms();
    if (st.iters > 0) st.vcycle_ms = vc_ms / st.iters;
    if (bdev && st.iters > 0) {
        int h = 0;
        IAMRX_HIP_CHECK(hipMemcpyAsync(&h, mg_bottom_iters_dev(), sizeof(int), hipMemcpyDeviceToHost, ctx.stream));
        ctx.sync();
        st.bottom_iters_total = h;
    }
    fillbc(0, phi);
    return st;
}

}
```

iamr_amd/csrc/operators.h:

```cpp
#pragma once
#include <string>
#include "mf.h"
#include "mlmg.h"
#include "kernels.h"
#include <memory>
#include <functional>

namespace iamrx {

MGStats mlmg_mac_solve(const Geometry& g, MultiFab* const umac[3], const MultiFab& rho, int rho_comp, const MultiFab* S,
                       MultiFab& mac_phi, double rhs_scale, const DomainBC& bc, double mac_tol, double mac_abs_tol,
                       const MGOpts& opts, MultiFab* const fluxes[3], const MultiFab* cphi = nullptr, const Geometry* cgeom = nullptr, int ratio = 2);

MGStats nodal_projection(const Geometry& g, MultiFab& vel, int vcomp, MultiFab& phi, const MultiFab& sig, int sig_comp,
                         const DomainBC& bc, double rel_tol, double abs_tol, const MGOpts& opts, MultiFab* gp, bool increment_gp,
                         const MultiFab* rhcc = nullptr );
void nodal_rhcc_add(const Geometry& g, MultiFab& rhs, const MultiFab& rc, const DomainBC& bc);
MultiFab make_rhcc(const Geometry& g, const MultiFab& src, int comp, double scale, const MultiFab* drop);
void mask_mult(MultiFab& y, int ycomp, int nc, const MultiFab& m, bool keep_where_zero, int ng);

MGStats level_project_single(const Geometry& g, double dt, MultiFab& U_new, int vcomp, MultiFab& P_new, const MultiFab& Gp_old, MultiFab& Gp_new,
                             const MultiFab& rho_half, const DomainBC& bc, double proj_tol, double proj_abs_tol, const MGOpts& opts);

struct TensorCF { const MultiFab* crse; const Geometry* cgeom; int ratio; };
struct TensorFlux { MultiFab* flux[3]; double fac; bool add; };
void tensor_apply(const Geometry& g, MultiFab& out, MultiFab& vel , double a_scalar, double b_scalar,
                  const MultiFab* acoef, const MultiFab* const eta[3], const DomainBC* bcs, int nbc ,
                  const TensorCF* cf = nullptr, const TensorFlux* fx = nullptr);
inline void tensor_apply(const Geometry& g, MultiFab& out, MultiFab& vel, double a_scalar, double b_scalar, const MultiFab* acoef,
                         const MultiFab* const eta[3], const DomainBC& bc) { tensor_apply(g, out, vel, a_scalar, b_scalar, acoef, eta, &bc, 1); }
MGStats tensor_solve(const Geometry& g, MultiFab& soln, const MultiFab& rhs, double a_scalar, double b_scalar, const MultiFab* acoef,
                     const MultiFab* const eta[3], const DomainBC* bcs, int nbc, double tol_rel, double tol_abs, const MGOpts& opts,
                     const TensorCF* cf = nullptr, const TensorFlux* fx = nullptr);
inline MGStats tensor_solve(const Geometry& g, MultiFab& soln, const MultiFab& rhs, double a_scalar, double b_scalar, const MultiFab* acoef,
                            const MultiFab* const eta[3], const DomainBC& bc, double tol_rel, double tol_abs, const MGOpts& opts)
{ return tensor_solve(g, soln, rhs, a_scalar, b_scalar, acoef, eta, &bc, 1, tol_rel, tol_abs, opts); }

void calc_mut_les(const Geometry& g, MultiFab& vel, const DomainBC bcs[3], int model, double Cs, double base, MultiFab* const mu[3],
                  const TensorCF* cf = nullptr);

struct DiffusionCrse { const MultiFab* crse_old; const MultiFab* crse_new; const Geometry* cgeom; int ratio; };
MGStats diffuse_scalar(const Geometry& g, const MultiFab* S_old, const MultiFab* Rho_old, MultiFab& S_new, const MultiFab* Rho_new, int sigma, int rho_comp, double dt, double theta,
                       const MultiFab& rho_half, int rho_flag, MultiFab* const fluxn[3], MultiFab* const fluxnp1[3],
                       const MultiFab* delta_rhs, int rhs_comp, const MultiFab* const betan[3], const MultiFab* const betanp1[3],
                       const DomainBC& bc, const DiffusionCrse* crse, bool add_old_time_divFlux, double visc_tol, const MGOpts& o);
MGStats diffuse_tensor_velocity(const Geometry& g, const MultiFab* U_old, MultiFab& U_new, int rho_comp, double dt, double theta,
                                const MultiFab& rho_half, int rho_flag, const MultiFab* visc_old_term, const MultiFab* const eta_n[3],
                                const MultiFab* const eta_np1[3], const DomainBC bc_visc[3], const DiffusionCrse* crse,
                                MultiFab* const tflux[3], double visc_tol, const MGOpts& o, const std::function<void(MultiFab&)>& fill_new);

MGStats diffuse_tensor_Vsync(const Geometry& g, MultiFab& Vsync, double dt, double theta, const MultiFab& rho_half, int rho_flag,
                             const MultiFab* Rho_old, const MultiFab* Rho_new, int rho_comp, const MultiFab* const eta[3],
                             const DomainBC bc_visc[3], const BCRec bc_vel[3], const Geometry* cgeom, int ratio, MultiFab* const tflux[3],
                             double visc_tol, const MGOpts& o);
MGStats diffuse_Ssync(const Geometry& g, MultiFab& Ssync, int sn, double dt, double theta, const MultiFab& rho_half, int rho_flag,
                      const MultiFab& Rho_new, int rho_comp, const MultiFab* const beta[3], const DomainBC& bc, const Geometry* cgeom, int ratio,
                      MultiFab* const flux[3], double visc_tol, const MGOpts& o);

class FluxRegister;
MGStats mac_sync_solve(const Geometry& g, FluxRegister& mr, const MultiFab& rho_half, double dt, LayoutP fine_layout, int ratio,
                       MultiFab* const Ucorr[3], MultiFab& mac_sync_phi, const DomainBC& bc, double tol, double abs_tol, const MGOpts& opts,
                       const Geometry* cgeom = nullptr, int cratio = 2);

void derive_mag_vort(const Geometry& g, MultiFab& out, int ocomp, const MultiFab& vel, int vcomp);
void error_tag(const Geometry& g, MultiFab& tags, const MultiFab& field, int comp, int mode, double value, int level,
               const double* rb_lo, const double* rb_hi);
struct OutflowTags { int nface = 0; int dir[6], side[6]; int mode = 0; int ncoarse = 0; };
void erode_map(std::vector<unsigned char>& m, const int n[3], const int per[3], int passes, const int lo[3], const int hi[3]);
std::vector<BoxD> cluster_tags(const unsigned char* tags_host, const BoxD& domain, int blocking_factor, int max_grid_size, double grid_eff,
                               int n_error_buf, const OutflowTags* oft = nullptr, const unsigned char* allowed = nullptr );

void parallel_copy(MultiFab& dst, const MultiFab& src, int scomp, int dcomp, int nc, int src_ng, int dst_ng, const Geometry* periodic_geom, bool add = false);
void relayout_copy(MultiFab& dst, const MultiFab& src, int nc, int scomp = 0, int dcomp = 0);
LayoutP merged_solve_layout(const Geometry& g, const LayoutP& l);
void average_down(const MultiFab& fine, MultiFab& crse, int scomp, int ncomp, int ratio);
struct TimeData { const MultiFab* old_; const MultiFab* new_; double t_old, t_new; };
const MultiFab* state_time_interp(const TimeData& td, double time, int scomp, int ncomp, MultiFab& tmp, int& comp0);
void fillpatch_two_levels(MultiFab& dst, int dcomp, double time, const TimeData& fine, const TimeData& crse, int scomp, int ncomp,
                          const Geometry& cgeom, const Geometry& fgeom, int ratio, const BCRec* bc, const double* extdir_lo, const double* extdir_hi);

void create_umac_grown(MultiFab* const umac_fine[3], const MultiFab* const umac_crse[3], const MultiFab* divu,
                       const Geometry& cgeom, const Geometry& fgeom, int ratio);
class FluxRegister {
public:
    FluxRegister(LayoutP fine, LayoutP crse, const Geometry& cgeom, int ratio, int ncomp);
    void setVal(double v);
    void CrseInit(const MultiFab& flux , int dir, int scomp, int dcomp, int nc, double mult, bool add);
    void FineAdd(const MultiFab& flux , int dir, int scomp, int dcomp, int nc, double mult);
    void Reflux(MultiFab& S , double volume, double scale, int scomp, int dcomp, int nc);
    const MultiFab& reg(int dir, int side) const { return m_reg[dir][side]; }
private:
    LayoutP m_fine, m_crse;
    Geometry m_cgeom;
    int m_ratio, m_ncomp;
    LayoutP m_slab[3][2];
    MultiFab m_reg[3][2];
};

void node_interp_from_crse(MultiFab& fine, const MultiFab& crse, const Geometry& cgeom, int ratio, const MultiFab* mask, bool add);
// ... 213 lines not shown
```

iamr_amd/csrc/projection.hip:

```cpp
#include "operators.h"
#include "launch.h"
#include <cstdlib>

namespace iamrx {

void nodal_rhcc_add(const Geometry& g, MultiFab& rhs, const MultiFab& rc, const DomainBC& bc)
{
    IAMRX_ASSERT(rc.ngrow >= 1);
    const FabD *rt = rhs.d_tab, *ct = rc.d_tab;
    const BoxD dom = g.domain;
    int nlo[3], nhi[3];
    for (int d = 0; d < 3; ++d) {
        nlo[d] = !g.periodic[d] && (bc.lo[d] == lo_neumann || bc.lo[d] == lo_inflow);
        nhi[d] = !g.periodic[d] && (bc.hi[d] == lo_neumann || bc.hi[d] == lo_inflow);
    }
    const int a0 = nlo[0], a1 = nlo[1], a2 = nlo[2], b0 = nhi[0], b1 = nhi[1], b2 = nhi[2];
    for_each(*rhs.layout, node_type(), 0, Context::get().stream, [=] __device__(int i, int j, int k, int f) {
        const FabD c = ct[f];
        double s = 0.0;
        for (int cz = 0; cz < 2; ++cz) for (int cy = 0; cy < 2; ++cy) for (int cx = 0; cx < 2; ++cx) s += c(i - 1 + cx, j - 1 + cy, k - 1 + cz);
        double r = 0.125 * s;
        if ((a0 && i == dom.lo[0]) || (b0 && i == dom.hi[0] + 1)) r *= 2.0;
        if ((a1 && j == dom.lo[1]) || (b1 && j == dom.hi[1] + 1)) r *= 2.0;
        if ((a2 && k == dom.lo[2]) || (b2 && k == dom.hi[2] + 1)) r *= 2.0;
        rt[f](i, j, k) += r;
    });
}

MultiFab make_rhcc(const Geometry& g, const MultiFab& src, int comp, double scale, const MultiFab* drop)
{
    MultiFab rc(src.layout, cell_type(), 1, 1);
    rc.setVal(0.0);
    MultiFab::Copy(rc, src, comp, 0, 1, 0);
    if (scale != 1.0) mf_mult(rc, scale, 0, 1, 0);
    if (drop) mask_mult(rc, 0, 1, *drop, true, 0);
    rc.FillBoundary(g);
    return rc;
}

MGStats nodal_projection(const Geometry& g, MultiFab& vel, int vcomp, MultiFab& phi, const MultiFab& sig, int sig_comp,
                         const DomainBC& bc, double rel_tol, double abs_tol, const MGOpts& opts, MultiFab* gp, bool increment_gp, const MultiFab* rhcc)
{
    LayoutP layout = phi.layout;
    if (LayoutP ml = merged_solve_layout(g, layout)) {
        MultiFab vel_m(ml, cell_type(), 3, vel.ngrow), phi_m(ml, node_type(), 1, phi.ngrow), sig_m(ml, cell_type(), 1, sig.ngrow), gp_m, rh_m;
        relayout_copy(vel_m, vel, 3, vcomp, 0);
        relayout_copy(phi_m, phi, 1);
        relayout_copy(sig_m, sig, 1, sig_comp, 0);
        if (gp) { gp_m.define(ml, cell_type(), 3, gp->ngrow); if (increment_gp) relayout_copy(gp_m, *gp, 3); }
        if (rhcc) { rh_m.define(ml, cell_type(), 1, rhcc->ngrow); relayout_copy(rh_m, *rhcc, 1); }
        MGStats st = nodal_projection(g, vel_m, 0, phi_m, sig_m, 0, bc, rel_tol, abs_tol, opts, gp ? &gp_m : nullptr, increment_gp, rhcc ? &rh_m : nullptr);
        relayout_copy(vel, vel_m, 3, 0, vcomp);
        relayout_copy(phi, phi_m, 1);
        if (gp) relayout_copy(*gp, gp_m, 3);
        return st;
    }
    vel.FillBoundary(g, vcomp, 3);
    NodalMG mg(g, layout, bc, opts);
    mg.setSigma(sig, sig_comp);
    MultiFab rhs(layout, node_type(), 1, 0);
    nodal_divu(g, rhs, vel, vcomp, &bc);
    if (rhcc) nodal_rhcc_add(g, rhs, *rhcc, bc);
    MGStats st = mg.solve(phi, rhs, rel_tol, abs_tol);
    nodal_mknewu(g, &vel, vcomp, phi, &mg.sigma(0), gp, increment_gp);
    if (gp) gp->FillBoundary(g);
    return st;
}

MGStats level_project_single(const Geometry& g, double dt, MultiFab& U_new, int vcomp, MultiFab& P_new, const MultiFab& Gp_old, MultiFab& Gp_new,
                             const MultiFab& rho_half, const DomainBC& bc, double proj_tol, double proj_abs_tol, const MGOpts& opts)
{
    LayoutP layout = P_new.layout;
    IAMRX_ASSERT(layout->total_cells() == g.domain.npts());
    P_new.setVal(0.0, 0, 1, 0);
    mf_mult(U_new, 1.0 / dt, vcomp, 3, 1);
    MultiFab sig(layout, cell_type(), 1, 1);
    {
        const FabD *nt = U_new.d_tab, *gt = Gp_old.d_tab, *ht = rho_half.d_tab, *st = sig.d_tab;
        for_each(*layout, cell_type(), 0, Context::get().stream, [=] __device__(int i, int j, int k, int f) {
            const double rh = ht[f](i, j, k, 0);
            for (int n = 0; n < 3; ++n) nt[f](i, j, k, vcomp + n) += gt[f](i, j, k, n) / rh;
            st[f](i, j, k, 0) = 1.0 / rh;
        });
    }
    MGStats st = nodal_projection(g, U_new, vcomp, P_new, sig, 0, bc, proj_tol, proj_abs_tol, opts, &Gp_new, false);
    mf_mult(U_new, dt, vcomp, 3, 1);
    return st;
}

static void setup_tensor(CellMG& mg, MultiFab tb[3], const MultiFab* bp[3], LayoutP layout, double a_scalar, double b_scalar,
                         const MultiFab* acoef, const MultiFab* const eta[3])
{
    const bool eta_form = tune("TENSOR_ETA", 1) != 0;
    for (int d = 0; d < 3; ++d) {
        if (eta_form) { bp[d] = eta[d]; continue; }
        tb[d].define(layout, face_type(d), 3, 0);
        tensor_bcoef(tb[d], *eta[d], d);
        bp[d] = &tb[d];
    }
    mg.setTensorEta(eta_form);
    mg.setScalars(a_scalar, b_scalar);
    if (acoef) mg.setACoeffs(acoef);
    mg.setBCoeffs(bp);
    mg.setTensor(true);
}

void tensor_apply(const Geometry& g, MultiFab& out, MultiFab& vel, double a_scalar, double b_scalar, const MultiFab* acoef,
                  const MultiFab* const eta[3], const DomainBC* bcs, int nbc, const TensorCF* cf, const TensorFlux* fx)
{
    MGOpts o;
    o.max_coarsening_level = 0;
    o.maxorder = bcs[0].maxorder;
    CellMG mg(g, vel.layout, 3, bcs[0], o);
    if (nbc > 1) mg.setDomainBCs(bcs, nbc);
    MultiFab tb[3];
    const MultiFab* bp[3];
    setup_tensor(mg, tb, bp, vel.layout, a_scalar, b_scalar, acoef, eta);
    if (cf) mg.setCoarseFineBC(cf->crse, *cf->cgeom, cf->ratio);
    mg.prepare();
    mg.apply(out, vel);
    if (fx) tensor_extensive_flux(g, vel, eta, fx->flux, fx->fac, fx->add);
}

MGStats tensor_solve(const Geometry& g, MultiFab& soln, const MultiFab& rhs, double a_scalar, double b_scalar, const MultiFab* acoef,
                     const MultiFab* const eta[3], const DomainBC* bcs, int nbc, double tol_rel, double tol_abs, const MGOpts& opts, const TensorCF* cf,
                     const TensorFlux* fx)
{
    MGOpts o = opts;
    o.maxorder = bcs[0].maxorder;
    CellMG mg(g, soln.layout, 3, bcs[0], o);
    if (nbc > 1) mg.setDomainBCs(bcs, nbc);
    MultiFab tb[3];
    const MultiFab* bp[3];
    setup_tensor(mg, tb, bp, soln.layout, a_scalar, b_scalar, acoef, eta);
    if (cf) mg.setCoarseFineBC(cf->crse, *cf->cgeom, cf->ratio);
    mg.prepare();
    MGStats st = mg.solve(soln, rhs, tol_rel, tol_abs);
    if (fx) tensor_extensive_flux(g, soln, eta, fx->flux, fx->fac, fx->add);
    return st;
}

void calc_mut_les(const Geometry& g, MultiFab& vel, const DomainBC bcs[3], int model, double Cs, double base, MultiFab* const mu[3], const TensorCF* cf)
{
    IAMRX_ASSERT(vel.ncomp == 3 && vel.ngrow >= 1);
    MGOpts o;
    o.max_coarsening_level = 0;
    o.maxorder = bcs[0].maxorder;
    CellMG mg(g, vel.layout, 3, bcs[0], o);
    mg.setDomainBCs(bcs, 3);
    mg.setTensor(true);
    if (cf) mg.setCoarseFineBC(cf->crse, *cf->cgeom, cf->ratio);
    mg.prepareBoundary();
    mg.fillBoundaryData(vel);
    les_mut(g, vel, 0, model, Cs, base, mu);
}

}
```

iamr_amd/ns.py:

```python
import ctypes as C
from .lib import lib, check, i3, mg_opts, MgStats, MultiFab, _h


class NsParams(C.Structure):
    _fields_ = [("cfl", C.c_double), ("visc_coef", C.c_double), ("be_cn_theta", C.c_double), ("gravity", C.c_double),
                ("mac_tol", C.c_double), ("mac_abs_tol", C.c_double), ("proj_tol", C.c_double),
                ("proj_abs_tol", C.c_double), ("visc_tol", C.c_double),
                ("use_forces_in_trans", C.c_int), ("do_mom_diff", C.c_int), ("init_iter", C.c_int),
                ("init_vel_iter", C.c_int), ("init_shrink", C.c_double), ("change_max", C.c_double),
                ("fixed_dt", C.c_double), ("nscal", C.c_int), ("verbose", C.c_int),
                ("init_dt", C.c_double), ("tracer_diff_coef", C.c_double), ("phys_lo", C.c_int * 3), ("phys_hi", C.c_int * 3),
                ("wall_vel_lo", C.c_double * 9), ("wall_vel_hi", C.c_double * 9),
                ("scal_bc_lo", C.c_double * 12), ("scal_bc_hi", C.c_double * 12), ("do_cons_trac", C.c_int), ("do_denminmax", C.c_int), ("do_scalminmax", C.c_int),
                ("do_trac2", C.c_int), ("do_cons_trac2", C.c_int), ("tracer2_diff_coef", C.c_double), ("do_temp", C.c_int), ("temp_cond_coef", C.c_double), ("use_ppm", C.c_int),
                ("avg_interval", C.c_int), ("compute_fluctuations", C.c_int), ("sum_interval", C.c_int),
                ("do_LES", C.c_int), ("LES_model", C.c_int), ("smago_Cs_cst", C.c_double), ("sigma_Cs_cst", C.c_double)]


def ns_params(**kw):
    p = NsParams()
    lib().iamrx_ns_default_params(C.byref(p))
    p.avg_in_checkpoint = int(kw.pop("avg_in_checkpoint", 1))
    for k, v in kw.items():
        if k in ("phys_lo", "phys_hi"):
            setattr(p, k, (C.c_int * 3)(*[int(x) for x in v]))
        elif k in ("wall_vel_lo", "wall_vel_hi"):
            setattr(p, k, (C.c_double * 9)(*[float(x) for x in v]))
        elif k in ("scal_bc_lo", "scal_bc_hi"):
            v = [float(x) for x in v]
            if len(v) == 6:
                v = [v[2 * d + n] if n < 2 else 0.0 for d in range(3) for n in range(4)]
            setattr(p, k, (C.c_double * 12)(*v))
        else:
            setattr(p, k, v)
    return p


def nodal_residual(geom, out, phi, sig, rhs=None):
    check(lib().iamrx_nodal_residual(C.byref(geom), out.h, phi.h, sig.h, _h(rhs)))


def nodal_gs_color(geom, phi, rhs, sig, color):
    check(lib().iamrx_nodal_gs_color(C.byref(geom), phi.h, rhs.h, sig.h, color))


def nodal_gs_sweep(geom, phi, rhs, sig, fused=1):
    check(lib().iamrx_nodal_gs_sweep(C.byref(geom), phi.h, rhs.h, sig.h, int(fused)))


def nodal_restrict(crse, fine):
    check(lib().iamrx_nodal_restrict(crse.h, fine.h))


def nodal_interp_add(fine, crse, sig_fine):
    check(lib().iamrx_nodal_interp_add(fine.h, crse.h, sig_fine.h))


def nodal_divu(geom, rhs, vel, vcomp=0):
    check(lib().iamrx_nodal_divu(C.byref(geom), rhs.h, vel.h, vcomp))


def nodal_compgrad(geom, gp, phi):
    check(lib().iamrx_nodal_compgrad(C.byref(geom), gp.h, phi.h))


def nodal_solve(geom, phi, rhs, sig, sig_comp=0, lobc=(0, 0, 0), hibc=(0, 0, 0), rel_tol=1e-12, abs_tol=1e-16, opts=None):
    st = MgStats()
    o = opts if opts is not None else mg_opts()
    check(lib().iamrx_nodal_solve(C.byref(geom), _h(phi), _h(rhs), _h(sig), sig_comp, i3(lobc), i3(hibc),
                                      C.c_double(rel_tol), C.c_double(abs_tol), C.byref(o), C.byref(st)))
    return st


def nodal_projection(geom, vel, vcomp, phi, sig, sig_comp=0, lobc=(0, 0, 0), hibc=(0, 0, 0), rel_tol=1e-12, abs_tol=1e-16,
                     opts=None, gp=None, increment_gp=False):
    st = MgStats()
    o = opts if opts is not None else mg_opts()
    check(lib().iamrx_nodal_projection(C.byref(geom), vel.h, vcomp, phi.h, sig.h, sig_comp, i3(lobc), i3(hibc),
                                       C.c_double(rel_tol), C.c_double(abs_tol), C.byref(o), _h(gp), int(increment_gp), C.byref(st)))
    return st


def _bcn(lobc, hibc):
    if hasattr(lobc[0], "__len__"):
        flat_lo = [int(v) for c in lobc for v in c]
        flat_hi = [int(v) for c in hibc for v in c]
        return (C.c_int * 9)(*flat_lo), (C.c_int * 9)(*flat_hi), 3
    return i3(lobc), i3(hibc), 1


def tensor_apply(geom, out, vel, a, b, acoef, eta, lobc=(0, 0, 0), hibc=(0, 0, 0), maxorder=2):
    lo, hi, nbc = _bcn(lobc, hibc)
    check(lib().iamrx_tensor_apply(C.byref(geom), out.h, vel.h, C.c_double(a), C.c_double(b), _h(acoef), eta[0].h, eta[1].h,
                                   eta[2].h, lo, hi, nbc, maxorder))


def tensor_solve(geom, soln, rhs, a, b, acoef, eta, lobc=(0, 0, 0), hibc=(0, 0, 0), tol_rel=1e-10, tol_abs=0.0, opts=None):
    st = MgStats()
    o = opts if opts is not None else mg_opts(maxorder=2)
    lo, hi, nbc = _bcn(lobc, hibc)
    check(lib().iamrx_tensor_solve(C.byref(geom), soln.h, rhs.h, C.c_double(a), C.c_double(b), _h(acoef), eta[0].h, eta[1].h,
                                   eta[2].h, lo, hi, nbc, C.c_double(tol_rel), C.c_double(tol_abs), C.byref(o), C.byref(st)))
    return st


def tensor_apply_cf(geom, out, vel, a, b, acoef, eta, crse_vel, cgeom, ratio=2, lobc=(0, 0, 0), hibc=(0, 0, 0), maxorder=2):
    lo, hi, nbc = _bcn(lobc, hibc)
    check(lib().iamrx_tensor_apply_cf(C.byref(geom), out.h, vel.h, C.c_double(a), C.c_double(b), _h(acoef), eta[0].h, eta[1].h,
                                      eta[2].h, lo, hi, nbc, maxorder, _h(crse_vel), C.byref(cgeom), int(ratio)))


def tensor_solve_cf(geom, soln, rhs, a, b, acoef, eta, crse_vel, cgeom, ratio=2, lobc=(0, 0, 0), hibc=(0, 0, 0), tol_rel=1e-10, tol_abs=0.0,
                    opts=None):
    st = MgStats()
    o = opts if opts is not None else mg_opts(maxorder=2)
    lo, hi, nbc = _bcn(lobc, hibc)
    check(lib().iamrx_tensor_solve_cf(C.byref(geom), soln.h, rhs.h, C.c_double(a), C.c_double(b), _h(acoef), eta[0].h, eta[1].h,
                                      eta[2].h, lo, hi, nbc, _h(crse_vel), C.byref(cgeom), int(ratio), C.c_double(tol_rel), C.c_double(tol_abs),
                                      C.byref(o), C.byref(st)))
    return st


SMAGORINSKY, SIGMA = 0, 1


def les_mut(geom, vel, mu, model, Cs, base=0.0, vcomp=0):
    check(lib().iamrx_les_mut(C.byref(geom), vel.h, int(vcomp), int(model), C.c_double(Cs), C.c_double(base), mu[0].h, mu[1].h, mu[2].h))


def calc_mut_les(geom, vel, mu, model, Cs, lobc=((0, 0, 0),) * 3, hibc=((0, 0, 0),) * 3, maxorder=3, crse_vel=None, cgeom=None, ratio=2):
    lo, hi, nbc = _bcn(lobc, hibc)
    assert nbc == 3
    if cgeom is None:
        check(lib().iamrx_calc_mut_les(C.byref(geom), vel.h, lo, hi, int(maxorder), int(model), C.c_double(Cs), mu[0].h, mu[1].h, mu[2].h))
    else:
        check(lib().iamrx_calc_mut_les_cf(C.byref(geom), vel.h, lo, hi, int(maxorder), int(model), C.c_double(Cs), mu[0].h, mu[1].h, mu[2].h,
                                          _h(crse_vel), C.byref(cgeom), int(ratio)))


class NavierStokes:
    S_NEW, S_OLD, P_NEW, P_OLD, GP_NEW, GP_OLD, UMAC_X, UMAC_Y, UMAC_Z, AOFS = range(10)
    ETA_N, ETA_NP1 = 13, 16
# ... 110 lines not shown
```

include/iamrx.h:

```cpp
#ifndef IAMRX_H
#define IAMRX_H
#include <stddef.h>

#ifdef __cplusplus
extern "C" {
#endif

typedef struct iamrx_layout_s* iamrx_layout;
typedef struct iamrx_fluxreg_s* iamrx_fluxreg;
typedef struct iamrx_mf_s* iamrx_mf;
typedef struct iamrx_ns_s* iamrx_ns;
typedef struct iamrx_syncreg_s* iamrx_syncreg;
typedef struct iamrx_amr_s* iamrx_amr;

typedef struct iamrx_geom {
    int dom_lo[3], dom_hi[3];
    double prob_lo[3], prob_hi[3];
    int periodic[3];
} iamrx_geom;

typedef struct iamrx_mg_opts {
    int nu1, nu2, nuf, nub;
    int max_iters, bottom_maxiter;
    double bottom_reltol;
// ... 45 lines not shown
int iamrx_comm_init_callback(int rank, int nranks, iamrx_allreduce_cb ar, iamrx_exchange_cb ex);
int iamrx_comm_rank(int* rank, int* nranks);
int iamrx_comm_allreduce(double* vals, int n, int op);
int iamrx_comm_probe_exchange(int peer, long count);
const char* iamrx_comm_last_error(void);

int iamrx_layout_create(int nboxes, const int* lo_hi , const int* owner_rank,
                        iamrx_layout* out);
int iamrx_layout_coalesced_boxes(iamrx_layout l, int* nboxes, int* lo_hi );
int iamrx_layout_destroy(iamrx_layout l);
int iamrx_layout_nlocal(iamrx_layout l, int* nlocal);
int iamrx_layout_local_box(iamrx_layout l, int local_idx, int lo_hi[6], int* global_idx);
int iamrx_layout_owners(iamrx_layout l, int* owners );
int iamrx_mf_create(iamrx_layout l, const int type[3] , int ncomp, int ngrow, iamrx_mf* out);
int iamrx_mf_destroy(iamrx_mf m);
int iamrx_mf_info(iamrx_mf m, int* ncomp, int* ngrow, int type[3], int* nlocal);
int iamrx_mf_fab_box(iamrx_mf m, int local_idx, int lo_hi[6]);
int iamrx_mf_dev_ptr(iamrx_mf m, int local_idx, double** p);
int iamrx_mf_to_host(iamrx_mf m, int local_idx, double* dst);
int iamrx_mf_from_host(iamrx_mf m, int local_idx, const double* src);
int iamrx_mf_setval(iamrx_mf m, double v);
int iamrx_mf_copy(iamrx_mf dst, iamrx_mf src, int scomp, int dcomp, int ncomp, int ngrow);
int iamrx_mf_fill_boundary(iamrx_mf m, const iamrx_geom* g);
int iamrx_mf_fill_physbc(iamrx_mf m, const iamrx_geom* g, int scomp, int ncomp, const int* bcrec, const double* extdir_lo,
                         const double* extdir_hi);
int iamrx_mf_norm0(iamrx_mf m, int comp, int ncomp, int ngrow, double* out);
int iamrx_mf_norm0_comps(iamrx_mf m, int comp, int ncomp, int ngrow, int form, double* out);
int iamrx_mf_minmax(iamrx_mf m, int comp, int ngrow, double* mn, double* mx);
int iamrx_mf_dot(const iamrx_geom* g, const int lobc[3], const int hibc[3], iamrx_mf x0, iamrx_mf y0, iamrx_mf x1, iamrx_mf y1, int comp,
                 int ncomp, int on_device, double out[2]);
int iamrx_mf_sum_unique(const iamrx_geom* g, const int lobc[3], const int hibc[3], iamrx_mf m, int comp, double* out);

int iamrx_host_fill_plan(int nboxes, const int* lo_hi, const int* owner, int rank, const int type[3], int ngrow, const iamrx_geom* g,
                         int max_desc, int* desc, int* ndesc);
int iamrx_host_fill_plan_wall_ext(int nboxes, const int* lo_hi, const int* owner, int rank, const int type[3], int ngrow, const iamrx_geom* g,
                                  int wall_ext, int max_desc, int* desc, int* ndesc);

int iamrx_host_abec_smoother_plan(int nboxes, const int* lo_hi, const iamrx_geom* g, const int lobc[3], const int hibc[3], int maxorder, int ncomp,
                                  int coef, int has_a, int has_cf, int finest, const int ngrow[4], int out[12]);

int iamrx_abec_gsrb(const iamrx_geom* g, double alpha, double beta, iamrx_mf a , iamrx_mf bx, iamrx_mf by, iamrx_mf bz,
                    iamrx_mf phi, iamrx_mf rhs, int redblack, double omega, const int lobc[3], const int hibc[3], int maxorder);
int iamrx_abec_form(const iamrx_geom* g, int coef, iamrx_mf rho, int rho_comp, double scale, const double bu[3], double beta, int op,
                    iamrx_mf phi, iamrx_mf rhs, iamrx_mf out, double omega, const int lobc[3], const int hibc[3], int maxorder);
int iamrx_abec_gsrb_sweep(const iamrx_geom* g, double alpha, double beta, iamrx_mf a , iamrx_mf bx, iamrx_mf by, iamrx_mf bz,
                          iamrx_mf phi, iamrx_mf rhs, double omega, const int lobc[3], const int hibc[3], int maxorder, int fused);
int iamrx_abec_residual(const iamrx_geom* g, double alpha, double beta, iamrx_mf a, iamrx_mf bx, iamrx_mf by, iamrx_mf bz,
                        iamrx_mf out, iamrx_mf phi, iamrx_mf rhs, int tensor);
int iamrx_cc_restrict(iamrx_mf crse, iamrx_mf fine);
int iamrx_cc_prolong_add(iamrx_mf fine, iamrx_mf crse);
int iamrx_face_avgdown(iamrx_mf crse, iamrx_mf fine, int dir);
int iamrx_abec_solve(const iamrx_geom* g, double alpha, double beta, iamrx_mf a, iamrx_mf bx, iamrx_mf by, iamrx_mf bz,
                     iamrx_mf phi, iamrx_mf rhs, const int lobc[3], const int hibc[3], double rtol, double atol,
                     const iamrx_mg_opts* o, int tensor, iamrx_mg_stats* st);

int iamrx_mlmg_mac_solve(const iamrx_geom* g, iamrx_mf umac_x, iamrx_mf umac_y, iamrx_mf umac_z, iamrx_mf rho, int rho_comp,
                         iamrx_mf S , iamrx_mf mac_phi, double rhs_scale, const int lobc[3], const int hibc[3],
                         double mac_tol, double mac_abs_tol, const iamrx_mg_opts* o, iamrx_mg_stats* st);
int iamrx_mlmg_mac_solve_cf(const iamrx_geom* g, iamrx_mf umac_x, iamrx_mf umac_y, iamrx_mf umac_z, iamrx_mf rho, int rho_comp,
                            iamrx_mf S , iamrx_mf mac_phi, double rhs_scale, const int lobc[3], const int hibc[3],
                            iamrx_mf crse_phi, const iamrx_geom* cgeom, int ratio, double mac_tol, double mac_abs_tol,
                            const iamrx_mg_opts* o, iamrx_mg_stats* st);
int iamrx_mac_sync_solve(const iamrx_geom* g, iamrx_fluxreg mac_reg, iamrx_mf rho_half, double dt, iamrx_layout fine, int ratio,
                         iamrx_mf ucorr_x, iamrx_mf ucorr_y, iamrx_mf ucorr_z, iamrx_mf mac_sync_phi, const int lobc[3], const int hibc[3],
                         double mac_sync_tol, double mac_abs_tol, const iamrx_mg_opts* o, iamrx_mg_stats* st);
int iamrx_mac_divergence(const iamrx_geom* g, iamrx_mf div, iamrx_mf umac_x, iamrx_mf umac_y, iamrx_mf umac_z);

#define IAMRX_GODUNOV_PLM 0
#define IAMRX_GODUNOV_PPM 1
#define IAMRX_BDS 2
int iamrx_godunov_extrap_vel_to_faces(const iamrx_geom* g, iamrx_mf vel, iamrx_mf force, iamrx_mf umac_x, iamrx_mf umac_y,
                                      iamrx_mf umac_z, double dt, const int* bcrec , int use_forces_in_trans, int scheme);
int iamrx_godunov_compute_aofs(const iamrx_geom* g, iamrx_mf aofs, int acomp, iamrx_mf S, int ncomp, iamrx_mf force, iamrx_mf divu,
                               iamrx_mf umac_x, iamrx_mf umac_y, iamrx_mf umac_z, const int* iconserv, double dt,
                               const int* bcrec , int is_velocity, int use_forces_in_trans,
                               iamrx_mf edge_x, iamrx_mf edge_y, iamrx_mf edge_z, iamrx_mf flux_x, iamrx_mf flux_y, iamrx_mf flux_z, int scheme);

int iamrx_nodal_residual(const iamrx_geom* g, iamrx_mf out, iamrx_mf phi, iamrx_mf sig, iamrx_mf rhs);
int iamrx_nodal_gs_color(const iamrx_geom* g, iamrx_mf phi, iamrx_mf rhs, iamrx_mf sig, int color);
int iamrx_nodal_gs_sweep(const iamrx_geom* g, iamrx_mf phi, iamrx_mf rhs, iamrx_mf sig, int fused);
int iamrx_nodal_restrict(iamrx_mf crse, iamrx_mf fine);
int iamrx_nodal_interp_add(iamrx_mf fine, iamrx_mf crse, iamrx_mf sig_fine);
int iamrx_nodal_divu(const iamrx_geom* g, iamrx_mf rhs, iamrx_mf vel, int vcomp);
int iamrx_nodal_compgrad(const iamrx_geom* g, iamrx_mf gp, iamrx_mf phi);
int iamrx_nodal_projection(const iamrx_geom* g, iamrx_mf vel, int vcomp, iamrx_mf phi, iamrx_mf sig, int sig_comp,
                           const int lobc[3], const int hibc[3], double rel_tol, double abs_tol, const iamrx_mg_opts* o,
                           iamrx_mf gp , int increment_gp, iamrx_mg_stats* st);

int iamrx_abec_solve_cf(const iamrx_geom* g, double alpha, double beta, iamrx_mf a, iamrx_mf bx, iamrx_mf by, iamrx_mf bz,
                        iamrx_mf phi, iamrx_mf rhs, const int lobc[3], const int hibc[3], iamrx_mf crse_phi, const iamrx_geom* cgeom,
                        int ratio, double rel_tol, double abs_tol, const iamrx_mg_opts* o, iamrx_mg_stats* st);

int iamrx_nodal_solve(const iamrx_geom* g, iamrx_mf phi, iamrx_mf rhs, iamrx_mf sig, int sig_comp, const int lobc[3], const int hibc[3],
                      double rel_tol, double abs_tol, const iamrx_mg_opts* o, iamrx_mg_stats* st);

int iamrx_tensor_apply(const iamrx_geom* g, iamrx_mf out, iamrx_mf vel, double a, double b, iamrx_mf acoef, iamrx_mf eta_x,
                       iamrx_mf eta_y, iamrx_mf eta_z, const int* lobc, const int* hibc, int nbc, int maxorder);
int iamrx_tensor_solve(const iamrx_geom* g, iamrx_mf soln, iamrx_mf rhs, double a, double b, iamrx_mf acoef, iamrx_mf eta_x,
                       iamrx_mf eta_y, iamrx_mf eta_z, const int* lobc, const int* hibc, int nbc, double tol_rel, double tol_abs,
                       const iamrx_mg_opts* o, iamrx_mg_stats* st);

int iamrx_tensor_extensive_flux(const iamrx_geom* g, iamrx_mf vel, iamrx_mf eta_x, iamrx_mf eta_y, iamrx_mf eta_z,
                                iamrx_mf flux_x, iamrx_mf flux_y, iamrx_mf flux_z, double fac, int add);
int iamrx_tensor_apply_cf(const iamrx_geom* g, iamrx_mf out, iamrx_mf vel, double a, double b, iamrx_mf acoef, iamrx_mf eta_x,
                          iamrx_mf eta_y, iamrx_mf eta_z, const int* lobc, const int* hibc, int nbc, int maxorder,
                          iamrx_mf crse_vel, const iamrx_geom* cgeom, int ratio);
int iamrx_tensor_solve_cf(const iamrx_geom* g, iamrx_mf soln, iamrx_mf rhs, double a, double b, iamrx_mf acoef, iamrx_mf eta_x,
                          iamrx_mf eta_y, iamrx_mf eta_z, const int* lobc, const int* hibc, int nbc, iamrx_mf crse_vel,
                          const iamrx_geom* cgeom, int ratio, double tol_rel, double tol_abs, const iamrx_mg_opts* o, iamrx_mg_stats* st);

int iamrx_les_mut(const iamrx_geom* g, iamrx_mf vel, int vcomp, int model, double Cs, double base, iamrx_mf mu_x, iamrx_mf mu_y, iamrx_mf mu_z);
int iamrx_calc_mut_les(const iamrx_geom* g, iamrx_mf vel, const int* lobc, const int* hibc, int maxorder, int model, double Cs,
                       iamrx_mf mu_x, iamrx_mf mu_y, iamrx_mf mu_z);
int iamrx_calc_mut_les_cf(const iamrx_geom* g, iamrx_mf vel, const int* lobc, const int* hibc, int maxorder, int model, double Cs,
                          iamrx_mf mu_x, iamrx_mf mu_y, iamrx_mf mu_z, iamrx_mf crse_vel, const iamrx_geom* cgeom, int ratio);

int iamrx_parallel_copy(iamrx_mf dst, iamrx_mf src, int scomp, int dcomp, int ncomp, int src_ng, int dst_ng, const iamrx_geom* periodic_geom);
int iamrx_average_down(iamrx_mf fine, iamrx_mf crse, int scomp, int ncomp, int ratio);
int iamrx_create_umac_grown(iamrx_mf umac_fine_x, iamrx_mf umac_fine_y, iamrx_mf umac_fine_z, iamrx_mf umac_crse_x, iamrx_mf umac_crse_y,
                            iamrx_mf umac_crse_z, iamrx_mf divu, const iamrx_geom* cgeom, const iamrx_geom* fgeom, int ratio);
int iamrx_fluxreg_create(iamrx_layout fine, iamrx_layout crse, const iamrx_geom* cgeom, int ratio, int ncomp, iamrx_fluxreg* out);
int iamrx_fluxreg_destroy(iamrx_fluxreg fr);
int iamrx_fluxreg_setval(iamrx_fluxreg fr, double v);
int iamrx_fluxreg_crse_init(iamrx_fluxreg fr, iamrx_mf crse_flux, int dir, int scomp, int dcomp, int ncomp, double mult, int add);
int iamrx_fluxreg_fine_add(iamrx_fluxreg fr, iamrx_mf fine_flux, int dir, int scomp, int dcomp, int ncomp, double mult);
int iamrx_fluxreg_reflux(iamrx_fluxreg fr, iamrx_mf S_crse, double volume, double scale, int scomp, int dcomp, int ncomp);
int iamrx_fillpatch_two_levels(iamrx_mf dst, int dcomp, double time, iamrx_mf fine_old, iamrx_mf fine_new, double t_fine_old, double t_fine_new,
                               iamrx_mf crse_old, iamrx_mf crse_new, double t_crse_old, double t_crse_new, int scomp, int ncomp,
                               const iamrx_geom* cgeom, const iamrx_geom* fgeom, int ratio, const int* bcrec, const double* extdir_lo, const double* extdir_hi);

int iamrx_derive_mag_vort(const iamrx_geom* g, iamrx_mf out, int ocomp, iamrx_mf vel, int vcomp);
int iamrx_error_tag(const iamrx_geom* g, iamrx_mf tags, iamrx_mf field, int comp, int mode, double value, int level,
                    const double* realbox_lo, const double* realbox_hi);
int iamrx_cluster_tags(const iamrx_geom* g, iamrx_mf tags, int blocking_factor, int max_grid_size, double grid_eff, int n_error_buf,
                       int* boxes, int* nboxes);
int iamrx_host_cluster_tags(const unsigned char* tags, const int dom_lo[3], const int dom_hi[3], int blocking_factor, int max_grid_size, double grid_eff,
                            int n_error_buf, const unsigned char* allowed, int* boxes, int* nboxes);
int iamrx_host_erode(unsigned char* map, const int n[3], const int periodic[3], int passes);

typedef struct iamrx_diffusion_crse { iamrx_mf crse_old, crse_new; const iamrx_geom* cgeom; int ratio; } iamrx_diffusion_crse;
int iamrx_diffuse_scalar(const iamrx_geom* g, iamrx_mf S_old, iamrx_mf Rho_old, iamrx_mf S_new, iamrx_mf Rho_new, int sigma, int rho_comp, double dt,
                         double be_cn_theta, iamrx_mf rho_half, int rho_flag, const iamrx_mf* fluxn, const iamrx_mf* fluxnp1, iamrx_mf delta_rhs,
                         int rhs_comp, const iamrx_mf* betan, const iamrx_mf* betanp1, const int* lobc, const int* hibc,
                         const iamrx_diffusion_crse* crse, int add_old_time_divFlux, double visc_tol, const iamrx_mg_opts* o, iamrx_mg_stats* st);
int iamrx_diffuse_tensor_velocity(const iamrx_geom* g, iamrx_mf U_old, iamrx_mf U_new, int rho_comp, double dt, double be_cn_theta, iamrx_mf rho_half,
                                  int rho_flag, iamrx_mf visc_old_term, const iamrx_mf* eta_n, const iamrx_mf* eta_np1, const int* lobc, const int* hibc,
                                  const iamrx_diffusion_crse* crse, const iamrx_mf* tflux, double visc_tol, const iamrx_mg_opts* o, iamrx_mg_stats* st,
                                  void (*fill_new)(void* ctx, iamrx_mf U_new), void* ctx);
int iamrx_diffuse_tensor_vsync(const iamrx_geom* g, iamrx_mf Vsync, double dt, double be_cn_theta, iamrx_mf rho_half, int rho_flag, iamrx_mf Rho_old,
                               iamrx_mf Rho_new, int rho_comp, const iamrx_mf* eta, const int* lobc, const int* hibc, const int* bcrec_vel,
                               const iamrx_geom* cgeom, int ratio, const iamrx_mf* tflux, double visc_tol, const iamrx_mg_opts* o, iamrx_mg_stats* st);
int iamrx_diffuse_ssync(const iamrx_geom* g, iamrx_mf Ssync, int comp, double dt, double be_cn_theta, iamrx_mf rho_half, int rho_flag, iamrx_mf Rho_new,
                        int rho_comp, const iamrx_mf* beta, const int* lobc, const int* hibc, const iamrx_geom* cgeom, int ratio, const iamrx_mf* flux,
                        double visc_tol, const iamrx_mg_opts* o, iamrx_mg_stats* st);

typedef struct iamrx_ns_params {
    double cfl, visc_coef, be_cn_theta, gravity;
    double mac_tol, mac_abs_tol, proj_tol, proj_abs_tol, visc_tol;
    int use_forces_in_trans, do_mom_diff, init_iter, init_vel_iter;
    double init_shrink, change_max, fixed_dt;
    int nscal, verbose;
    double init_dt;
    double tracer_diff_coef;
    int phys_lo[3], phys_hi[3];
    double wall_vel_lo[9], wall_vel_hi[9];
    double scal_bc_lo[12], scal_bc_hi[12];
// ... 110 lines not shown
```

Measured before the change: 470.3 million cells/s.

## Tile nodal restrict/divu in shared memory, fuse projection scaling, skip redundant fills

Adds shared-memory z-marching kernels for nodal restriction and nodal divergence so neighboring fine/cell values are reused from LDS instead of re-read from global memory. Folds the post-projection dt velocity scaling into the mknewu update and only scales ghost cells separately. Lets the nodal MG solve reuse the temporary RHS in place instead of copying it, and skips zero-initialising level arrays that are fully written first. Also adds a BC-aware divu C/Python entry point. Each path sits behind a tune flag and carries correctness risk at boundaries and ghost regions.

```diff
diff --git a/iamr_amd/csrc/cabi.hip b/iamr_amd/csrc/cabi.hip
--- a/iamr_amd/csrc/cabi.hip
+++ b/iamr_amd/csrc/cabi.hip
@@ -671,6 +671,13 @@
     nodal_divu(gg, rhs->mf, vel->mf, vcomp, &bc);
     IAMRX_CATCH
 }
+int iamrx_nodal_divu_bc(const iamrx_geom* g, iamrx_mf rhs, iamrx_mf vel, int vcomp, const int lobc[3], const int hibc[3])
+{
+    IAMRX_TRY
+    const DomainBC bc = to_bc(lobc, hibc, 2);
+    nodal_divu(to_geom(g), rhs->mf, vel->mf, vcomp, &bc);
+    IAMRX_CATCH
+}
 int iamrx_nodal_compgrad(const iamrx_geom* g, iamrx_mf gp, iamrx_mf phi)
 {
     IAMRX_TRY nodal_mknewu(to_geom(g), nullptr, 0, phi->mf, nullptr, &gp->mf, false); IAMRX_CATCH
diff --git a/iamr_amd/csrc/k_basic.hip b/iamr_amd/csrc/k_basic.hip
--- a/iamr_amd/csrc/k_basic.hip
+++ b/iamr_amd/csrc/k_basic.hip
@@ -1,5 +1,6 @@
 #include "kernels.h"
 #include "launch.h"
+#include <algorithm>
 
 namespace iamrx {
 
@@ -505,6 +506,48 @@
         [=] __device__(int i, int j, int k, int f, int n, double v) { yt[f](i, j, k, comp + n) = v; });
 }
 
+__global__ void __launch_bounds__(256) k_mult_shell(const BoxD* __restrict__ boxes, const FabD* __restrict__ yt, int t0, int t1, int t2, int ng, int comp, int nc, double a)
+{
+    const int fab = blockIdx.y;
+    BoxD b = boxes[fab];
+    b.hi[0] += t0; b.hi[1] += t1; b.hi[2] += t2;
+    const FabD y = yt[fab];
+    const long nx = b.len(0), ny = b.len(1), nz = b.len(2), gx = nx + 2 * ng, gy = ny + 2 * ng;
+    const long nA = gx * gy * ng, nB = gx * ng * nz, nC = ng * ny * nz;
+    const long total = 2 * (nA + nB + nC);
+    for (long idx = (long)blockIdx.x * 256 + threadIdx.x; idx < total; idx += (long)gridDim.x * 256) {
+        long r = idx;
+        int i, j, k;
+        if (r < 2 * nA) {
+            const int side = (int)(r / nA); r -= side * nA;
+            i = b.lo[0] - ng + (int)(r % gx); j = b.lo[1] - ng + (int)((r / gx) % gy);
+            k = (side ? b.hi[2] + 1 : b.lo[2] - ng) + (int)(r / (gx * gy));
+        } else if ((r -= 2 * nA) < 2 * nB) {
+            const int side = (int)(r / nB); r -= side * nB;
+            i = b.lo[0] - ng + (int)(r % gx); k = b.lo[2] + (int)(r / (gx * ng));
+            j = (side ? b.hi[1] + 1 : b.lo[1] - ng) + (int)((r / gx) % ng);
+        } else {
+            r -= 2 * nB;
+            const int side = (int)(r / nC); r -= side * nC;
+            j = b.lo[1] + (int)((r / ng) % ny); k = b.lo[2] + (int)(r / (ng * ny));
+            i = (side ? b.hi[0] + 1 : b.lo[0] - ng) + (int)(r % ng);
+        }
+        for (int n = 0; n < nc; ++n) y(i, j, k, comp + n) = y(i, j, k, comp + n) * a;
+    }
+}
+
+void mf_mult_ghosts(MultiFab& y, double a, int comp, int nc, int ng)
+{
+    if (!y.base || ng <= 0 || y.nlocal() == 0) return;
+    IAMRX_ASSERT(ng <= y.ngrow);
+    const Layout& l = *y.layout;
+    const long nx = l.max_len[0] + y.type.t[0], ny = l.max_len[1] + y.type.t[1], nz = l.max_len[2] + y.type.t[2];
+    const long total = 2 * ((nx + 2 * ng) * (ny + 2 * ng) * ng + (nx + 2 * ng) * ng * nz + ng * ny * nz);
+    const long nb = std::min<long>((total + 255) / 256, 4096);
+    hipLaunchKernelGGL(k_mult_shell, dim3((unsigned)nb, (unsigned)l.nlocal()), dim3(256), 0, Context::get().stream, l.d_boxes, y.d_tab, y.type.t[0], y.type.t[1],
+                       y.type.t[2], ng, comp, nc, a);
+}
+
 void slab_duplicate(MultiFab& dst, const MultiFab& src)
 {
     IAMRX_ASSERT(dst.ncomp == src.ncomp && dst.layout->boxes.size() == src.layout->boxes.size());
diff --git a/iamr_amd/csrc/k_nodal.hip b/iamr_amd/csrc/k_nodal.hip
--- a/iamr_amd/csrc/k_nodal.hip
+++ b/iamr_amd/csrc/k_nodal.hip
@@ -1406,10 +1406,98 @@
     });
 }
 
+template <int CTX, int CTY>
+__global__ void __launch_bounds__(CTX * CTY) k_nodal_restrict_tile(const BoxD* __restrict__ cboxes, const FabD* __restrict__ ct, const FabD* __restrict__ ft,
+    int ntx, int nty, int kc)
+{
+    constexpr int FX = 2 * CTX + 1, FY = 2 * CTY + 1, HX = CTX + 1, PX = 2 * HX, NT = CTX * CTY, NLD = (FX * FY + NT - 1) / NT;
+    __shared__ double F[3][FY][PX];
+    const int fab = blockIdx.y;
+    const BoxD cb = cboxes[fab];
+    const int bid = blockIdx.x;
+    const int tix = bid % ntx, r1 = bid / ntx, tiy = r1 % nty, ck = r1 / nty;
+    const int nhi0 = cb.hi[0] + 1, nhi1 = cb.hi[1] + 1, nhi2 = cb.hi[2] + 1;
+    const int i0 = cb.lo[0] + tix * CTX, j0 = cb.lo[1] + tiy * CTY, k0 = cb.lo[2] + ck * kc;
+    if (i0 > nhi0 || j0 > nhi1 || k0 > nhi2) return;
+    const int k1 = min(k0 + kc - 1, nhi2);
+    const FabD fa = ft[fab], c = ct[fab];
+    const int ox = 2 * i0 - 1, oy = 2 * j0 - 1;
+    const int tid = threadIdx.x;
+    long foff[NLD];
+    int lslot[NLD];
+    const int fhi0 = min(2 * nhi0 + 1, fa.lo[0] + fa.n[0] - 1), fhi1 = min(2 * nhi1 + 1, fa.lo[1] + fa.n[1] - 1);
+#pragma unroll
+    for (int it = 0; it < NLD; ++it) {
+        const int idx = tid + it * NT;
+        const int lx = idx % FX, ly = idx / FX;
+        const int gi = ox + lx, gj = oy + ly;
+        const bool on = idx < FX * FY && gi >= fa.lo[0] && gi <= fhi0 && gj >= fa.lo[1] && gj <= fhi1;
+        foff[it] = on ? fa.off(gi, gj, fa.lo[2]) : -1;
+        lslot[it] = idx < FX * FY ? ly * PX + (lx & 1) * HX + (lx >> 1) : -1;
+    }
+    const long fpl = (long)fa.n[0] * fa.n[1];
+    const FabD::gdouble* fp = (const FabD::gdouble*)fa.p;
+    const int fklo = fa.lo[2], fkhi = fa.lo[2] + fa.n[2] - 1;
+    auto ldf = [&](int it, int k) { return (foff[it] >= 0 && k >= fklo && k <= fkhi) ? (double)fp[foff[it] + fpl * (k - fklo)] : 0.0; };
+    double* Fl = &F[0][0][0];
+    constexpr int PL = FY * PX;
+    int sm = 0, s0 = 1, sp = 2;
+    double v0[NLD], v1[NLD];
+#pragma unroll
+    for (int it = 0; it < NLD; ++it) {
+        const double vm = ldf(it, 2 * k0 - 1);
+        v0[it] = ldf(it, 2 * k0); v1[it] = ldf(it, 2 * k0 + 1);
+        if (lslot[it] >= 0) Fl[sm * PL + lslot[it]] = vm;
+    }
+    const int tx = tid % CTX, ty = tid / CTX;
+    const int i = i0 + tx, j = j0 + ty;
+    const bool valid = i <= nhi0 && j <= nhi1;
+    const int cxm = tx, cx0 = HX + tx, cxp = tx + 1;
+    for (int k = k0; k <= k1; ++k) {
+#pragma unroll
+        for (int it = 0; it < NLD; ++it)
+            if (lslot[it] >= 0) { Fl[s0 * PL + lslot[it]] = v0[it]; Fl[sp * PL + lslot[it]] = v1[it]; }
+        __syncthreads();
+        if (k < k1) {
+#pragma unroll
+            for (int it = 0; it < NLD; ++it) { v0[it] = ldf(it, 2 * k + 2); v1[it] = ldf(it, 2 * k + 3); }
+        }
+        if (valid) {
+            const int pl[3] = {sm, s0, sp};
+            double s = 0.0;
+#pragma unroll
+            for (int dk = 0; dk < 3; ++dk)
+#pragma unroll
+                for (int dj = 0; dj < 3; ++dj) {
+                    const double* row = Fl + pl[dk] * PL + (2 * ty + dj) * PX;
+                    const double wjk = (dj == 1 ? 2. : 1.) * (dk == 1 ? 2. : 1.);
+                    s += (1. * wjk) * row[cxm];
+                    s += (2. * wjk) * row[cx0];
+                    s += (1. * wjk) * row[cxp];
+                }
+            c(i, j, k) = s * (1. / 64.);
+        }
+        __syncthreads();
+        const int t = sm; sm = sp; sp = s0; s0 = t;
+    }
+}
+
 void nodal_restrict(MultiFab& crse, const MultiFab& fine)
 {
     if (crse.nlocal() == 0) return;
     const FabD *ct = crse.d_tab, *ft = fine.d_tab;
+    const Layout& cl = *crse.layout;
+    const int min_x = std::max(16, (int)tune("NODAL_RESTRICT_MIN", 48));
+    if (tune("NODAL_RESTRICT_TILE", 1) != 0 && cl.max_len[0] >= min_x && cl.max_len[1] >= 8 && fine.ngrow >= 1) {
+        constexpr int CTX = 32, CTY = 8;
+        const int ntx = (cl.max_len[0] + 1 + CTX - 1) / CTX, nty = (cl.max_len[1] + 1 + CTY - 1) / CTY;
+        const int nk = cl.max_len[2] + 1;
+        const int kc = nk >= 64 ? 8 : 4;
+        const int nck = (nk + kc - 1) / kc;
+        dim3 grid((unsigned)(ntx * nty * nck), (unsigned)cl.nlocal());
+        hipLaunchKernelGGL((k_nodal_restrict_tile<CTX, CTY>), grid, dim3(CTX * CTY), 0, Context::get().stream, cl.d_boxes, ct, ft, ntx, nty, kc);
+        return;
+    }
     for_each(*crse.layout, node_type(), 0, Context::get().stream, [=] __device__(int i, int j, int k, int f) {
         const FabD fa = ft[f];
         const int ii = 2 * i, jj = 2 * j, kk = 2 * k;
@@ -1592,45 +1680,139 @@
     });
 }
 
+struct DivuGeom {
+    int wl[3], wh[3], il[3], ih[3];
+    int dl[3], dh[3];
+    double f[3];
+};
+
+template <class V>
+__device__ __forceinline__ double divu_node(const DivuGeom& G, int i, int j, int k, const V& v)
+{
+    double sx = 0.0, sy = 0.0, sz = 0.0;
+#pragma unroll
+    for (int cz = 0; cz < 2; ++cz)
+#pragma unroll
+        for (int cy = 0; cy < 2; ++cy)
+#pragma unroll
+            for (int cx = 0; cx < 2; ++cx) {
+                const int ci = i - 1 + cx, cj = j - 1 + cy, ck = k - 1 + cz;
+                const bool outside = (G.wl[0] && ci < G.dl[0]) || (G.wh[0] && ci > G.dh[0]) || (G.wl[1] && cj < G.dl[1]) || (G.wh[1] && cj > G.dh[1]) ||
+                                     (G.wl[2] && ck < G.dl[2]) || (G.wh[2] && ck > G.dh[2]);
+                const bool in0 = (G.il[0] && ci < G.dl[0]) || (G.ih[0] && ci > G.dh[0]), in1 = (G.il[1] && cj < G.dl[1]) || (G.ih[1] && cj > G.dh[1]),
+                           in2 = (G.il[2] && ck < G.dl[2]) || (G.ih[2] && ck > G.dh[2]);
+                sx += (cx ? 1.0 : -1.0) * ((outside || in1 || in2) ? 0.0 : v(ci, cj, ck, 0));
+                sy += (cy ? 1.0 : -1.0) * ((outside || in0 || in2) ? 0.0 : v(ci, cj, ck, 1));
+                sz += (cz ? 1.0 : -1.0) * ((outside || in0 || in1) ? 0.0 : v(ci, cj, ck, 2));
+            }
+    double r = 0.0;
+    r += G.f[0] * sx; r += G.f[1] * sy; r += G.f[2] * sz;
+    if ((G.wl[0] || G.il[0]) && i == G.dl[0]) r *= 2.0;
+    if ((G.wh[0] || G.ih[0]) && i == G.dh[0] + 1) r *= 2.0;
+    if ((G.wl[1] || G.il[1]) && j == G.dl[1]) r *= 2.0;
+    if ((G.wh[1] || G.ih[1]) && j == G.dh[1] + 1) r *= 2.0;
+    if ((G.wl[2] || G.il[2]) && k == G.dl[2]) r *= 2.0;
+    if ((G.wh[2] || G.ih[2]) && k == G.dh[2] + 1) r *= 2.0;
+    return r;
+}
+
+template <int TX, int TY>
+__global__ void __launch_bounds__(TX * TY) k_nodal_divu_zm(const BoxD* __restrict__ boxes, const FabD* __restrict__ rt, const FabD* __restrict__ vt, int vcomp,
+    DivuGeom G, int ntx, int nty, int kc)
+{
+    constexpr int RX = TX + 1, RY = TY + 1, NT = TX * TY, NLD = (RX * RY + NT - 1) / NT;
+    __shared__ double V[2][3][RY][RX];
+    const int fab = blockIdx.y;
+    const BoxD cb = boxes[fab];
+    const int bid = blockIdx.x;
+    const int tix = bid % ntx, r1 = bid / ntx, tiy = r1 % nty, ck = r1 / nty;
+    const int nhi0 = cb.hi[0] + 1, nhi1 = cb.hi[1] + 1, nhi2 = cb.hi[2] + 1;
+    const int tx0 = cb.lo[0] + tix * TX, ty0 = cb.lo[1] + tiy * TY, k0 = cb.lo[2] + ck * kc;
+    if (tx0 > nhi0 || ty0 > nhi1 || k0 > nhi2) return;
+    const int k1 = min(k0 + kc - 1, nhi2);
+    const FabD v = vt[fab], o = rt[fab];
+    const int ox = tx0 - 1, oy = ty0 - 1;
+    const int tid = threadIdx.x;
+    long voff[NLD];
+    int lidx[NLD];
+    const int chi0 = min(nhi0, v.lo[0] + v.n[0] - 1), chi1 = min(nhi1, v.lo[1] + v.n[1] - 1);
+#pragma unroll
+    for (int it = 0; it < NLD; ++it) {
+        const int idx = tid + it * NT;
+        const int gi = ox + idx % RX, gj = oy + idx / RX;
+        const bool on = idx < RX * RY && gi >= v.lo[0] && gi <= chi0 && gj >= v.lo[1] && gj <= chi1;
+        voff[it] = on ? v.off(gi, gj, v.lo[2]) + v.cs * vcomp : -1;
+        lidx[it] = idx < RX * RY ? idx : -1;
+    }
+    const long vpl = (long)v.n[0] * v.n[1];
+    const FabD::gdouble* vp = (const FabD::gdouble*)v.p;
+    const int vklo = v.lo[2], vkhi = v.lo[2] + v.n[2] - 1;
+    auto ldv = [&](int it, int n, int k) { return (voff[it] >= 0 && k >= vklo && k <= vkhi) ? (double)vp[voff[it] + v.cs * n + vpl * (k - vklo)] : 0.0; };
+    double* Vl = &V[0][0][0][0];
+    constexpr int PC = RY * RX, PL = 3 * PC;
+    double nv[NLD][3];
+#pragma unroll
+    for (int it = 0; it < NLD; ++it)
+#pragma unroll
+        for (int n = 0; n < 3; ++n) {
+            const double vm = ldv(it, n, k0 - 1);
+            nv[it][n] = ldv(it, n, k0);
+            if (lidx[it] >= 0) Vl[((k0 + 1) & 1) * PL + n * PC + lidx[it]] = vm;
+        }
+    const int lx = tid % TX + 1, ly = tid / TX + 1;
+    const int i = ox + lx, j = oy + ly;
+    const bool valid = i <= nhi0 && j <= nhi1;
+    for (int k = k0; k <= k1; ++k) {
+#pragma unroll
+        for (int it = 0; it < NLD; ++it)
+#pragma unroll
+            for (int n = 0; n < 3; ++n)
+                if (lidx[it] >= 0) Vl[(k & 1) * PL + n * PC + lidx[it]] = nv[it][n];
+        __syncthreads();
+        if (k < k1) {
+#pragma unroll
+            for (int it = 0; it < NLD; ++it)
+#pragma unroll
+                for (int n = 0; n < 3; ++n) nv[it][n] = ldv(it, n, k + 1);
+        }
+        if (valid) {
+            o(i, j, k) = divu_node(G, i, j, k, [&](int ci, int cj, int ck, int n) { return Vl[(ck & 1) * PL + n * PC + (cj - oy) * RX + (ci - ox)]; });
+        }
+        __syncthreads();
+    }
+}
+
 void nodal_divu(const Geometry& g, MultiFab& rhs, const MultiFab& vel, int vcomp, const DomainBC* bc)
 {
     if (rhs.nlocal() == 0) return;
     const FabD *rt = rhs.d_tab, *vt = vel.d_tab;
-    const double fx = 0.25 / g.dx[0], fy = 0.25 / g.dx[1], fz = 0.25 / g.dx[2];
-    int wl[3], wh[3], il[3], ih[3];
+    DivuGeom G;
     for (int d = 0; d < 3; ++d) {
-        wl[d] = (bc && !g.periodic[d] && bc->lo[d] == lo_neumann) ? 1 : 0;
-        wh[d] = (bc && !g.periodic[d] && bc->hi[d] == lo_neumann) ? 1 : 0;
-        il[d] = (bc && !g.periodic[d] && bc->lo[d] == lo_inflow) ? 1 : 0;
-        ih[d] = (bc && !g.periodic[d] && bc->hi[d] == lo_inflow) ? 1 : 0;
-    }
-    const int wl0 = wl[0], wl1 = wl[1], wl2 = wl[2], wh0 = wh[0], wh1 = wh[1], wh2 = wh[2];
-    const int il0 = il[0], il1 = il[1], il2 = il[2], ih0 = ih[0], ih1 = ih[1], ih2 = ih[2];
-    const int dl0 = g.domain.lo[0], dl1 = g.domain.lo[1], dl2 = g.domain.lo[2], dh0 = g.domain.hi[0], dh1 = g.domain.hi[1], dh2 = g.domain.hi[2];
-    for_each(*rhs.layout, node_type(), 0, Context::get().stream, [=] __device__(int i, int j, int k, int f) {
+        G.wl[d] = (bc && !g.periodic[d] && bc->lo[d] == lo_neumann) ? 1 : 0;
+        G.wh[d] = (bc && !g.periodic[d] && bc->hi[d] == lo_neumann) ? 1 : 0;
+        G.il[d] = (bc && !g.periodic[d] && bc->lo[d] == lo_inflow) ? 1 : 0;
+        G.ih[d] = (bc && !g.periodic[d] && bc->hi[d] == lo_inflow) ? 1 : 0;
+        G.dl[d] = g.domain.lo[d]; G.dh[d] = g.domain.hi[d];
+        G.f[d] = 0.25 / g.dx[d];
+    }
+    const Layout& l = *rhs.layout;
+    if (tune("NODAL_DIVU_ZM", 1) != 0 && l.max_len[0] >= 16 && l.max_len[1] >= 8 && vel.ngrow >= 1) {
+        constexpr int TX = 32, TY = 8;
+        const int ntx = (l.max_len[0] + 1 + TX - 1) / TX, nty = (l.max_len[1] + 1 + TY - 1) / TY;
+        const int nk = l.max_len[2] + 1;
+        const int kc = nk >= 128 ? 32 : (nk >= 32 ? 16 : nk);
+        const int nck = (nk + kc - 1) / kc;
+        dim3 grid((unsigned)(ntx * nty * nck), (unsigned)l.nlocal());
+        hipLaunchKernelGGL((k_nodal_divu_zm<TX, TY>), grid, dim3(TX * TY), 0, Context::get().stream, l.d_boxes, rt, vt, vcomp, G, ntx, nty, kc);
+        return;
+    }
+    for_each(l, node_type(), 0, Context::get().stream, [=] __device__(int i, int j, int k, int f) {
         const FabD v = vt[f];
-        double sx = 0.0, sy = 0.0, sz = 0.0;
-        for (int cz = 0; cz < 2; ++cz) for (int cy = 0; cy < 2; ++cy) for (int cx = 0; cx < 2; ++cx) {
-            const int ci = i - 1 + cx, cj = j - 1 + cy, ck = k - 1 + cz;
-            const bool outside = (wl0 && ci < dl0) || (wh0 && ci > dh0) || (wl1 && cj < dl1) || (wh1 && cj > dh1) || (wl2 && ck < dl2) || (wh2 && ck > dh2);
-            const bool in0 = (il0 && ci < dl0) || (ih0 && ci > dh0), in1 = (il1 && cj < dl1) || (ih1 && cj > dh1), in2 = (il2 && ck < dl2) || (ih2 && ck > dh2);
-            sx += (cx ? 1.0 : -1.0) * ((outside || in1 || in2) ? 0.0 : v(ci, cj, ck, vcomp));
-            sy += (cy ? 1.0 : -1.0) * ((outside || in0 || in2) ? 0.0 : v(ci, cj, ck, vcomp + 1));
-            sz += (cz ? 1.0 : -1.0) * ((outside || in0 || in1) ? 0.0 : v(ci, cj, ck, vcomp + 2));
-        }
-        double r = 0.0;
-        r += fx * sx; r += fy * sy; r += fz * sz;
-        if ((wl0 || il0) && i == dl0) r *= 2.0;
-        if ((wh0 || ih0) && i == dh0 + 1) r *= 2.0;
-        if ((wl1 || il1) && j == dl1) r *= 2.0;
-        if ((wh1 || ih1) && j == dh1 + 1) r *= 2.0;
-        if ((wl2 || il2) && k == dl2) r *= 2.0;
-        if ((wh2 || ih2) && k == dh2 + 1) r *= 2.0;
-        rt[f](i, j, k) = r;
+        rt[f](i, j, k) = divu_node(G, i, j, k, [&](int ci, int cj, int ck, int n) { return (double)v(ci, cj, ck, vcomp + n); });
     });
 }
 
-void nodal_mknewu(const Geometry& g, MultiFab* vel, int vcomp, const MultiFab& phi, const MultiFab* sig, MultiFab* gp, bool gp_increment)
+void nodal_mknewu(const Geometry& g, MultiFab* vel, int vcomp, const MultiFab& phi, const MultiFab* sig, MultiFab* gp, bool gp_increment, double vel_scale)
 {
     if (phi.nlocal() == 0) return;
     const FabD* pt = phi.d_tab;
@@ -1652,7 +1834,12 @@
         if (vt) {
             const double sg = st[f](i, j, k);
             const double fc[3] = {f0, f1, f2};
-            for (int d = 0; d < 3; ++d) vt[f](i, j, k, vcomp + d) -= sg * fc[d] * s[d];
+            for (int d = 0; d < 3; ++d) {
+                double u = vt[f](i, j, k, vcomp + d);
+                u -= sg * fc[d] * s[d];
+                if (vel_scale != 1.0) u = u * vel_scale;
+                vt[f](i, j, k, vcomp + d) = u;
+            }
         }
         if (gt) for (int d = 0; d < 3; ++d) { if (gp_increment) gt[f](i, j, k, d) += gr[d]; else gt[f](i, j, k, d) = gr[d]; }
     });
diff --git a/iamr_amd/csrc/kernels.h b/iamr_amd/csrc/kernels.h
--- a/iamr_amd/csrc/kernels.h
+++ b/iamr_amd/csrc/kernels.h
@@ -30,6 +30,7 @@
 void mf_saxpy(MultiFab& y, double a, const MultiFab& x, int xcomp, int ycomp, int nc, int ng);
 void mf_add_scalar(MultiFab& y, double a, int comp, int nc, int ng);
 void mf_mult(MultiFab& y, double a, int comp, int nc, int ng);
+void mf_mult_ghosts(MultiFab& y, double a, int comp, int nc, int ng);
 
 void stats_accumulate(MultiFab& avg, const MultiFab& S, int vcomp, double dt_avg, double t_sum, bool fluct);
 void stats_derive_vel_avg(MultiFab& out, int ocomp, const MultiFab& avg, double t_mean, double t_fluct);
@@ -156,7 +157,7 @@
 void nodal_restrict(MultiFab& crse, const MultiFab& fine);
 void nodal_interp_add(MultiFab& fine, const MultiFab& crse, const MultiFab& sig_fine);
 void nodal_divu(const Geometry& g, MultiFab& rhs, const MultiFab& vel, int vcomp, const DomainBC* bc);
-void nodal_mknewu(const Geometry& g, MultiFab* vel, int vcomp, const MultiFab& phi, const MultiFab* sig, MultiFab* gp, bool gp_increment);
+void nodal_mknewu(const Geometry& g, MultiFab* vel, int vcomp, const MultiFab& phi, const MultiFab* sig, MultiFab* gp, bool gp_increment, double vel_scale = 1.0);
 
 void tensor_bcoef(MultiFab& b3, const MultiFab& eta, int dir);
 void tensor_extensive_flux(const Geometry& g, const MultiFab& vel, const MultiFab* const eta[3], MultiFab* const flux[3], double fac, bool add);
diff --git a/iamr_amd/csrc/mlmg.h b/iamr_amd/csrc/mlmg.h
--- a/iamr_amd/csrc/mlmg.h
+++ b/iamr_amd/csrc/mlmg.h
@@ -185,7 +185,7 @@
 public:
     NodalMG(const Geometry& g, LayoutP layout, const DomainBC& bc, const MGOpts& o);
     void setSigma(const MultiFab& sig, int comp);
-    MGStats solve(MultiFab& phi, const MultiFab& rhs, double rtol, double atol);
+    MGStats solve(MultiFab& phi, const MultiFab& rhs, double rtol, double atol, bool rhs_is_temporary = false);
     int nlevels() const { return (int)m_lev.size(); }
     bool masked() const { return m_masked; }
     const MultiFab* dmask(int l) const { return m_lev[l].dmask(); }
diff --git a/iamr_amd/csrc/navierstokes.hip b/iamr_amd/csrc/navierstokes.hip
--- a/iamr_amd/csrc/navierstokes.hip
+++ b/iamr_amd/csrc/navierstokes.hip
@@ -1131,7 +1131,9 @@
         rhcc = make_rhcc(g, rhv, 0, 1.0, nullptr);
     }
     const MultiFab* rv = have_divu ? &rhv : nullptr;
-    st_nodal = nodal_projection(g, Sn, Xvel, Pn, sig, 0, bc_nodal, p.proj_tol, p.proj_abs_tol, o, &Gp[pnew], false, have_divu ? &rhcc : nullptr);
+    const bool fused_scale = tune("PROJ_SCALE_FUSED", 1) != 0;
+    st_nodal = nodal_projection(g, Sn, Xvel, Pn, sig, 0, bc_nodal, p.proj_tol, p.proj_abs_tol, o, &Gp[pnew], false, have_divu ? &rhcc : nullptr,
+                                fused_scale ? dt_ : 1.0);
     fill_gradp_bc();
     if (want_crse) {
         MultiFab r = amr_sync_resid(*this, vold, Pn, sig, true, rv);
@@ -1141,7 +1143,8 @@
         MultiFab r = amr_sync_resid(*this, vold, Pn, sig, false, rv);
         sync_reg->FineAdd(r, 1.0 / (double)ncycle);
     }
-    mf_mult(Sn, dt_, Xvel, 3, 1);
+    if (fused_scale) mf_mult_ghosts(Sn, dt_, Xvel, 3, 1);
+    else mf_mult(Sn, dt_, Xvel, 3, 1);
 }
 
 void NavierStokes::set_inflow_ghosts(MultiFab& vel, double scale)
diff --git a/iamr_amd/csrc/nodalmg.hip b/iamr_amd/csrc/nodalmg.hip
--- a/iamr_amd/csrc/nodalmg.hip
+++ b/iamr_amd/csrc/nodalmg.hip
@@ -49,20 +49,24 @@
         if (!mg_coarsen_level(f, m_o, c)) break;
         m_lev.push_back(std::move(c));
     }
+    bool need_mask = false;
+    for (int d = 0; d < 3; ++d) if (!g.periodic[d] && (bc.lo[d] == lo_dirichlet || bc.hi[d] == lo_dirichlet)) need_mask = true;
+    if (m_lev[0].layout->total_cells() != g.domain.npts()) need_mask = true;
     for (auto& L : m_lev) {
         if (L.agg) L.tmp_d.define(L.dist, node_type(), 1, 1);
         if (L.slab) L.vres.define(L.virt, node_type(), 1, 0);
         const int ng = nodal_fused() ? 4 : 1;
         L.sig.define(L.layout, cell_type(), 1, ng);
-        L.sig.setVal(0.0);
         L.cor.define(L.layout, node_type(), 1, ng);
         L.res.define(L.layout, node_type(), 1, ng);
         L.rescor.define(L.layout, node_type(), 1, 1);
+        int refl = 0;
+        const bool written_first = tune("NODAL_SKIP_FILLS", 1) != 0 && !need_mask && m_o.nodal_smoother == 0 && nodal_fused() &&
+                                   nodal_wrap_or_reflect_ok(L.g, *L.layout, m_bc, 4, &refl) && nodal_gsr_applies(L.cor, L.res, nullptr);
+        if (written_first) continue;
+        L.sig.setVal(0.0);
         L.cor.setVal(0.0); L.res.setVal(0.0); L.rescor.setVal(0.0);
     }
-    bool need_mask = false;
-    for (int d = 0; d < 3; ++d) if (!g.periodic[d] && (bc.lo[d] == lo_dirichlet || bc.hi[d] == lo_dirichlet)) need_mask = true;
-    if (m_lev[0].layout->total_cells() != g.domain.npts()) need_mask = true;
     for (auto& L : m_lev) {
         if (!need_mask) break;
         MultiFab cov(L.layout, cell_type(), 1, 1);
@@ -306,15 +310,20 @@
     nodal_reflect_bc(L0.g, L0.cor, m_bc);
 }
 
-MGStats NodalMG::solve(MultiFab& phi, const MultiFab& rhs_in, double rtol, double atol)
+MGStats NodalMG::solve(MultiFab& phi, const MultiFab& rhs_in, double rtol, double atol, bool rhs_is_temporary)
 {
     ProfScope ps_prof_("nmg_solve");
     auto& ctx = Context::get();
     MGStats st;
     st.nlevels = (int)m_lev.size();
     Level& L0 = m_lev[0];
-    MultiFab rhs(L0.layout, node_type(), 1, 0);
-    MultiFab::Copy(rhs, rhs_in, 0, 0, 1, 0);
+    const bool inplace = rhs_is_temporary && tune("NODAL_RHS_INPLACE", 1) != 0;
+    MultiFab rhs_copy;
+    if (!inplace) {
+        rhs_copy.define(L0.layout, node_type(), 1, 0);
+        MultiFab::Copy(rhs_copy, rhs_in, 0, 0, 1, 0);
+    }
+    MultiFab& rhs = inplace ? const_cast<MultiFab&>(rhs_in) : rhs_copy;
     if (L0.dmask()) nodal_zero_masked(rhs, L0.dm);
     if (m_singular) subtract_mean(0, rhs);
     residual(0, L0.res, phi, rhs, &st.resnorm0);
diff --git a/iamr_amd/csrc/operators.h b/iamr_amd/csrc/operators.h
--- a/iamr_amd/csrc/operators.h
+++ b/iamr_amd/csrc/operators.h
@@ -14,7 +14,8 @@
 
 MGStats nodal_projection(const Geometry& g, MultiFab& vel, int vcomp, MultiFab& phi, const MultiFab& sig, int sig_comp,
                          const DomainBC& bc, double rel_tol, double abs_tol, const MGOpts& opts, MultiFab* gp, bool increment_gp,
-                         const MultiFab* rhcc = nullptr );
+                         const MultiFab* rhcc = nullptr ,
+                         double vel_scale = 1.0 );
 void nodal_rhcc_add(const Geometry& g, MultiFab& rhs, const MultiFab& rc, const DomainBC& bc);
 MultiFab make_rhcc(const Geometry& g, const MultiFab& src, int comp, double scale, const MultiFab* drop);
 void mask_mult(MultiFab& y, int ycomp, int nc, const MultiFab& m, bool keep_where_zero, int ng);
diff --git a/iamr_amd/csrc/projection.hip b/iamr_amd/csrc/projection.hip
--- a/iamr_amd/csrc/projection.hip
+++ b/iamr_amd/csrc/projection.hip
@@ -39,7 +39,8 @@
 }
 
 MGStats nodal_projection(const Geometry& g, MultiFab& vel, int vcomp, MultiFab& phi, const MultiFab& sig, int sig_comp,
-                         const DomainBC& bc, double rel_tol, double abs_tol, const MGOpts& opts, MultiFab* gp, bool increment_gp, const MultiFab* rhcc)
+                         const DomainBC& bc, double rel_tol, double abs_tol, const MGOpts& opts, MultiFab* gp, bool increment_gp, const MultiFab* rhcc,
+                         double vel_scale)
 {
     LayoutP layout = phi.layout;
     if (LayoutP ml = merged_solve_layout(g, layout)) {
@@ -51,6 +52,7 @@
         if (rhcc) { rh_m.define(ml, cell_type(), 1, rhcc->ngrow); relayout_copy(rh_m, *rhcc, 1); }
         MGStats st = nodal_projection(g, vel_m, 0, phi_m, sig_m, 0, bc, rel_tol, abs_tol, opts, gp ? &gp_m : nullptr, increment_gp, rhcc ? &rh_m : nullptr);
         relayout_copy(vel, vel_m, 3, 0, vcomp);
+        if (vel_scale != 1.0) mf_mult(vel, vel_scale, vcomp, 3, 0);
         relayout_copy(phi, phi_m, 1);
         if (gp) relayout_copy(*gp, gp_m, 3);
         return st;
@@ -61,8 +63,8 @@
     MultiFab rhs(layout, node_type(), 1, 0);
     nodal_divu(g, rhs, vel, vcomp, &bc);
     if (rhcc) nodal_rhcc_add(g, rhs, *rhcc, bc);
-    MGStats st = mg.solve(phi, rhs, rel_tol, abs_tol);
-    nodal_mknewu(g, &vel, vcomp, phi, &mg.sigma(0), gp, increment_gp);
+    MGStats st = mg.solve(phi, rhs, rel_tol, abs_tol, true);
+    nodal_mknewu(g, &vel, vcomp, phi, &mg.sigma(0), gp, increment_gp, vel_scale);
     if (gp) gp->FillBoundary(g);
     return st;
 }
@@ -83,8 +85,10 @@
             st[f](i, j, k, 0) = 1.0 / rh;
         });
     }
-    MGStats st = nodal_projection(g, U_new, vcomp, P_new, sig, 0, bc, proj_tol, proj_abs_tol, opts, &Gp_new, false);
-    mf_mult(U_new, dt, vcomp, 3, 1);
+    const bool fused_scale = tune("PROJ_SCALE_FUSED", 1) != 0;
+    MGStats st = nodal_projection(g, U_new, vcomp, P_new, sig, 0, bc, proj_tol, proj_abs_tol, opts, &Gp_new, false, nullptr, fused_scale ? dt : 1.0);
+    if (fused_scale) mf_mult_ghosts(U_new, dt, vcomp, 3, 1);
+    else mf_mult(U_new, dt, vcomp, 3, 1);
     return st;
 }
 
diff --git a/iamr_amd/ns.py b/iamr_amd/ns.py
--- a/iamr_amd/ns.py
+++ b/iamr_amd/ns.py
@@ -56,8 +56,11 @@
     check(lib().iamrx_nodal_interp_add(fine.h, crse.h, sig_fine.h))
 
 
-def nodal_divu(geom, rhs, vel, vcomp=0):
-    check(lib().iamrx_nodal_divu(C.byref(geom), rhs.h, vel.h, vcomp))
+def nodal_divu(geom, rhs, vel, vcomp=0, lobc=None, hibc=None):
+    if lobc is None and hibc is None:
+        check(lib().iamrx_nodal_divu(C.byref(geom), rhs.h, vel.h, vcomp))
+    else:
+        check(lib().iamrx_nodal_divu_bc(C.byref(geom), rhs.h, vel.h, vcomp, i3(lobc), i3(hibc)))
 
 
 def nodal_compgrad(geom, gp, phi):
diff --git a/include/iamrx.h b/include/iamrx.h
--- a/include/iamrx.h
+++ b/include/iamrx.h
@@ -151,6 +151,7 @@
 int iamrx_nodal_restrict(iamrx_mf crse, iamrx_mf fine);
 int iamrx_nodal_interp_add(iamrx_mf fine, iamrx_mf crse, iamrx_mf sig_fine);
 int iamrx_nodal_divu(const iamrx_geom* g, iamrx_mf rhs, iamrx_mf vel, int vcomp);
+int iamrx_nodal_divu_bc(const iamrx_geom* g, iamrx_mf rhs, iamrx_mf vel, int vcomp, const int lobc[3], const int hibc[3]);
 int iamrx_nodal_compgrad(const iamrx_geom* g, iamrx_mf gp, iamrx_mf phi);
 int iamrx_nodal_projection(const iamrx_geom* g, iamrx_mf vel, int vcomp, iamrx_mf phi, iamrx_mf sig, int sig_comp,
                            const int lobc[3], const int hibc[3], double rel_tol, double abs_tol, const iamrx_mg_opts* o,
```

Result: faster. 481.2 million cells/s, median of 6 (+2.3%).
